# refresh-bio/vclust

Hardware: AMD Instinct MI355X
Metric: genome pairs/sec through prefilter+align (ani.tsv) (higher is better)
Workload: dtype u64

## Files before the change

### include/vclust_gpu.h

```cpp
#ifndef VCLUST_GPU_H
#define VCLUST_GPU_H

#include <stdint.h>

#ifdef __cplusplus
extern "C" {
#endif

enum {
    VG_OK = 0, VG_EINVAL = -1, VG_EIO = -2, VG_ENODEV = -3, VG_EHIP = -4, VG_ENOMEM = -5,
    VG_EOVERFLOW = -6
};

const char* vg_version(void);
const char* vg_last_error(void);
void        vg_free(void* p);
int vg_device_count(void);
int vg_set_device(int device);
void vg_release_device_memory(void);
int vg_alloc_selftest(const int64_t* sizes, int n_sizes, int cycles);
int vg_copy(void* dst, const void* src, int64_t bytes, int to_host);

typedef struct vg_genomes vg_genomes;

int vg_genomes_load(const char* const* paths, int n_paths, int multisample, int n_threads,
                    vg_genomes** out);
int vg_genomes_load_db_new(const char* const* db_paths, int n_db, const char* const* new_paths, int n_new, int multisample,
                           int n_threads, vg_genomes** out, int* n_db_genomes);
int vg_genomes_from_codes(const uint8_t* codes, const int64_t* offsets, int n_genomes,
                          const char* const* names, vg_genomes** out);
void        vg_genomes_free(vg_genomes* g);
int         vg_genomes_count(const vg_genomes* g);
int64_t     vg_genomes_total_len(const vg_genomes* g);
int         vg_genomes_lengths(const vg_genomes* g, int64_t* out );
const char* vg_genomes_name(const vg_genomes* g, int idx);
int         vg_genomes_codes(const vg_genomes* g, int idx, uint8_t* out);
int vg_genomes_to_device(vg_genomes* g);

typedef struct { uint32_t a, b, shared; } vg_pair_count;

int vg_kmer_shared(vg_genomes* g, int k, double fraction, int shard, int n_shards,
                   uint32_t min_shared, int64_t* set_sizes, vg_pair_count** pairs,
                   int64_t* n_pairs);
int vg_kmer_shared_new(vg_genomes* g, int n_db, int k, double fraction, uint32_t min_shared, int64_t* set_sizes,
                       vg_pair_count** pairs, int64_t* n_pairs);
void vg_set_new_path(int mode);
typedef struct {
    int accepted; int64_t P; int n_passes;
    int levels, total_bits, B1, B2;
    int st_tiles; int64_t n_st; int u_st, g_st;
    int tile32k, narrow, short_rec;
} vg_kmer_geometry_info;
int vg_kmer_geometry(const vg_genomes* g, int k, double fraction, int shard, int n_shards, vg_kmer_geometry_info* info);
int vg_kmer_geometry_at(int64_t padded_positions, int k, vg_kmer_geometry_info* info);
int vg_rowptr_inline_lo(int64_t entries, int64_t n_genomes, uint32_t* inline_lo);
int vg_kmer_set(vg_genomes* g, int idx, int k, double fraction, uint64_t** out, int64_t* n_out);

int vg_write_fltr(const vg_genomes* g, int k, double fraction, int min_kmers, double min_ident,
                  int max_seqs, const int64_t* set_sizes, const vg_pair_count* pairs,
                  int64_t n_pairs, const char* out_path);

int vg_filter_pairs(int k, int min_kmers, double min_ident, const int64_t* set_sizes, int64_t n_genomes,
                    const vg_pair_count* pairs, int64_t n_pairs, vg_pair_count** out, int64_t* n_out);

typedef struct {
    int    k;
    int    min_kmers;
    double min_ident;
    int    batch_size;
    double kmers_fraction;
    int    max_seqs;
    int    num_threads;
    int    verbosity;
    int    is_multifasta;
} vg_prefilter_params;
int vg_prefilter(const char* const* fasta_paths, int n_paths, const char* out_path,
                 const vg_prefilter_params* p);
int vg_prefilter_new(const char* const* db_paths, int n_db_paths, const char* const* new_paths, int n_new_paths,
                     const char* out_path, const vg_prefilter_params* p);
void vg_set_process_ends_after_call(int on);

typedef struct { int mal, msl, mrd, mqd, reg, aw, am, ar; } vg_lz_params;
typedef struct { uint32_t q, r; } vg_task;
typedef struct { uint32_t n_match, aln_len, n_regions; } vg_pair_stat;
typedef struct {
    uint32_t task; int32_t qstart, qend, rstart, rend; int32_t n_match;
} vg_region;

typedef struct { int weak_seed_ratio, anchor_margin, seed_choice; } vg_lz_fit;
void vg_set_lz_fit(const vg_lz_fit* f);

int vg_lz_align(vg_genomes* g, const vg_task* tasks, int64_t n_tasks, const vg_lz_params* p,
                vg_pair_stat* stats, vg_region** regions, int64_t* n_regions);

int vg_lz_prepare(vg_genomes* g, const vg_pair_count* pairs, int64_t n_pairs, const vg_lz_params* p);

int vg_align_order(const vg_genomes* g, int32_t* order );
int vg_read_filter(const vg_genomes* g, const char* path, double thr,
                   vg_pair_count** pairs, int64_t* n_pairs);

int vg_align_tasks(const vg_genomes* g, const vg_pair_count* pairs, int64_t n_pairs,
                   vg_task** tasks, int64_t* n_tasks);
int vg_lz_index_dump(vg_genomes* g, int idx, const vg_lz_params* p,
                     uint32_t** bucket_end, uint32_t** entries, int64_t* n_entries,
                     int* pos_bits, int* tag_bits, int* path);
void vg_set_index_budget(int64_t bytes);
void vg_set_subshards(int n);
void vg_set_range_scan(int mode);
void vg_set_placement_trials(int n);

typedef struct {
    vg_lz_params lz;
    double out_tani, out_gani, out_ani, out_qcov, out_rcov;
    const char* filter_path; double filter_threshold;
    const char* out_aln_path;
    const char* const* out_columns; int n_out_columns;
    int num_threads; int verbosity; int is_multifasta;
} vg_align_params;
int vg_write_ani(const vg_genomes* g, const vg_task* tasks, const vg_pair_stat* stats,
                 int64_t n_tasks, const vg_region* regions, int64_t n_regions,
                 const char* out_path, const vg_align_params* p);
int vg_align(const char* const* fasta_paths, int n_paths, const char* out_path,
             const vg_align_params* p);

int vg_align_new(const char* const* db_paths, int n_db_paths, const char* const* new_paths, int n_new_paths,
                 const char* out_path, const vg_align_params* p);

typedef struct vg_comm vg_comm;
typedef int (*vg_allgather_fn)(void* ctx, const void* send, void* recv, int64_t bytes, int on_device);
int  vg_comm_create(int rank, int world, vg_allgather_fn allgather, void* ctx, vg_comm** out);
int  vg_rccl_unique_id(void* out , int64_t bytes);
int  vg_comm_rccl_create(int rank, int world, const void* unique_id, int64_t id_bytes, vg_comm** out);
void vg_comm_free(vg_comm* c);
int  vg_comm_kind(const vg_comm* c);
int  vg_comm_rccl_ranks(const vg_comm* c);
int  vg_comm_rank(const vg_comm* c);
int  vg_comm_world(const vg_comm* c);
int  vg_comm_selftest(const vg_comm* c, int64_t bytes);
int vg_kmer_shared_sharded(vg_genomes* g, int k, double fraction, uint32_t min_shared, const vg_comm* c,
                           int64_t* set_sizes, vg_pair_count** pairs, int64_t* n_pairs);
int vg_align_owner(const vg_task* tasks, int64_t n_tasks, int n_genomes, int world, int32_t* owner );
int vg_lz_align_sharded(vg_genomes* g, const vg_task* tasks, int64_t n_tasks, const vg_lz_params* p, const vg_comm* c,
                        vg_pair_stat* stats, vg_region** regions, int64_t* n_regions);
int vg_align_pairs_share(const vg_genomes* g, const vg_pair_count* pairs, int64_t n_pairs, int world, int rank,
                         vg_task** tasks, int64_t* n_tasks);
int vg_lz_align_pairs_sharded(vg_genomes* g, const vg_pair_count* pairs, int64_t n_pairs, const vg_lz_params* p, const vg_comm* c,
                              vg_task** tasks, int64_t* n_tasks, vg_pair_stat** stats);
int vg_prefilter_sharded(const char* const* fasta_paths, int n_paths, const char* out_path,
                         const vg_prefilter_params* p, const vg_comm* c);
int vg_align_sharded(const char* const* fasta_paths, int n_paths, const char* out_path,
                     const vg_align_params* p, const vg_comm* c);

enum { VG_CLUSTER_SINGLE = 0, VG_CLUSTER_CDHIT = 1, VG_CLUSTER_UCLUST = 2, VG_CLUSTER_SET_COVER = 3, VG_CLUSTER_COMPLETE = 4, VG_CLUSTER_AVERAGE = 5,
       VG_CLUSTER_MCL = 6  };
typedef struct {
    int algorithm;
    const char* metric;
    double min_tani, min_gani, min_ani, min_qcov, min_rcov, min_len_ratio;
    int max_num_alns;
    int representatives;
    int num_threads; int verbosity;
} vg_cluster_params;
typedef struct {
    int64_t rounds;
    int64_t sweep_objects;
    int64_t n_edges;
} vg_cluster_stats;
int vg_cluster(const char* ani_path, const char* ids_path, const char* out_path, const vg_cluster_params* p);
int vg_cluster_graph(int64_t n_objects, const uint32_t* q, const uint32_t* r, const double* w, int64_t n_edges,
                     int algorithm, int32_t* label, int32_t* representative, vg_cluster_stats* stats);

typedef struct {
    int64_t rounds, sweep_objects, n_edges;
    int64_t n_prior, n_new;
    int64_t joined_prior, joined_new, founded;
    int64_t prior_merged;
} vg_cluster_update_stats;
int vg_cluster_update_graph(int64_t n_objects, const uint32_t* q, const uint32_t* r, const double* w, int64_t n_rows,
                            int algorithm, const int32_t* prior_rep, int32_t* label, int32_t* representative,
                            vg_cluster_update_stats* stats);
int vg_cluster_update(const char* ani_path, const char* ids_path, const char* prior_path, int prior_is_repr,
                      const char* out_path, const vg_cluster_params* p, vg_cluster_update_stats* stats);

typedef struct {
    int64_t rounds;
// ... 132 lines not shown
```

### vclust_amd/_lib.py

```python
import ctypes as C
import pathlib

PKG_DIR = pathlib.Path(__file__).resolve().parent
LIB_PATH = PKG_DIR / 'libvclust_gpu.so'


class VclustGpuError(RuntimeError):
    def __init__(self, code, msg):
        super().__init__(f'libvclust_gpu error {code}: {msg}')
        self.code = code


class PairCount(C.Structure):
    _fields_ = [('a', C.c_uint32), ('b', C.c_uint32), ('shared', C.c_uint32)]


class Task(C.Structure):
    _fields_ = [('q', C.c_uint32), ('r', C.c_uint32)]


class PairStat(C.Structure):
    _fields_ = [('n_match', C.c_uint32), ('aln_len', C.c_uint32), ('n_regions', C.c_uint32)]


# ... 65 lines not shown

class MclStats(C.Structure):
    _fields_ = [(name, C.c_int64) for name in ('iterations', 'converged', 'n_edges', 'nnz', 'max_row_seen', 'lds_rows', 'spill_rows')] + [('chaos', C.c_uint64)]


class DedupParams(C.Structure):
    _fields_ = [('gzip_level', C.c_int), ('num_threads', C.c_int), ('verbosity', C.c_int)]


class DedupStats(C.Structure):
    _fields_ = [('records', C.c_int64), ('unique', C.c_int64), ('removed', C.c_int64), ('reverse', C.c_int64),
                ('rounds', C.c_int64), ('collisions', C.c_int64)]


class DedupOptions(C.Structure):
    _fields_ = [('circular', C.c_int)]


class DedupContainedStats(C.Structure):
    _fields_ = [('passes', C.c_int64), ('positions', C.c_int64), ('hits', C.c_int64), ('candidates', C.c_int64),
                ('verified', C.c_int64), ('slices', C.c_int64)]


class DedupRepeatStats(C.Structure):
    _fields_ = [('with_repeat', C.c_int64), ('repeat_symbols', C.c_int64), ('candidates', C.c_int64), ('equal', C.c_int64),
                ('batches', C.c_int64)]


class KmerGeometry(C.Structure):
    _fields_ = [('accepted', C.c_int), ('P', C.c_int64), ('n_passes', C.c_int),
                ('levels', C.c_int), ('total_bits', C.c_int), ('B1', C.c_int), ('B2', C.c_int),
                ('st_tiles', C.c_int), ('n_st', C.c_int64), ('u_st', C.c_int), ('g_st', C.c_int),
                ('tile32k', C.c_int), ('narrow', C.c_int), ('short_rec', C.c_int)]


class KernelTime(C.Structure):
    _fields_ = [('name', C.c_char * 48), ('total_ms', C.c_double), ('launches', C.c_int64),
                ('bytes', C.c_double)]


ALLGATHER_FN = C.CFUNCTYPE(C.c_int, C.c_void_p, C.c_void_p, C.c_void_p, C.c_int64, C.c_int)

P = C.POINTER
SYMBOLS = {
    'vg_version': (C.c_char_p, []),
    'vg_last_error': (C.c_char_p, []),
    'vg_free': (None, [C.c_void_p]),
    'vg_device_count': (C.c_int, []),
    'vg_set_device': (C.c_int, [C.c_int]),
    'vg_release_device_memory': (None, []),
    'vg_copy': (C.c_int, [C.c_void_p, C.c_void_p, C.c_int64, C.c_int]),
    'vg_alloc_selftest': (C.c_int, [C.POINTER(C.c_int64), C.c_int, C.c_int]),
    'vg_genomes_load': (C.c_int, [P(C.c_char_p), C.c_int, C.c_int, C.c_int, P(C.c_void_p)]),
    'vg_genomes_load_db_new': (C.c_int, [P(C.c_char_p), C.c_int, P(C.c_char_p), C.c_int, C.c_int, C.c_int, P(C.c_void_p), P(C.c_int)]),
    'vg_genomes_from_codes': (C.c_int, [C.c_void_p, C.c_void_p, C.c_int, P(C.c_char_p), P(C.c_void_p)]),
    'vg_genomes_free': (None, [C.c_void_p]),
    'vg_genomes_count': (C.c_int, [C.c_void_p]),
    'vg_genomes_total_len': (C.c_int64, [C.c_void_p]),
    'vg_genomes_lengths': (C.c_int, [C.c_void_p, P(C.c_int64)]),
    'vg_genomes_name': (C.c_char_p, [C.c_void_p, C.c_int]),
    'vg_genomes_codes': (C.c_int, [C.c_void_p, C.c_int, C.c_void_p]),
    'vg_genomes_to_device': (C.c_int, [C.c_void_p]),
    'vg_kmer_shared': (C.c_int, [C.c_void_p, C.c_int, C.c_double, C.c_int, C.c_int, C.c_uint32,
                                 P(C.c_int64), P(P(PairCount)), P(C.c_int64)]),
    'vg_kmer_shared_new': (C.c_int, [C.c_void_p, C.c_int, C.c_int, C.c_double, C.c_uint32, P(C.c_int64), P(P(PairCount)), P(C.c_int64)]),
    'vg_kmer_geometry': (C.c_int, [C.c_void_p, C.c_int, C.c_double, C.c_int, C.c_int, P(KmerGeometry)]),
    'vg_kmer_geometry_at': (C.c_int, [C.c_int64, C.c_int, P(KmerGeometry)]),
    'vg_rowptr_inline_lo': (C.c_int, [C.c_int64, C.c_int64, P(C.c_uint32)]),
    'vg_kmer_set': (C.c_int, [C.c_void_p, C.c_int, C.c_int, C.c_double, P(P(C.c_uint64)), P(C.c_int64)]),
    'vg_filter_pairs': (C.c_int, [C.c_int, C.c_int, C.c_double, C.POINTER(C.c_int64), C.c_int64, C.POINTER(PairCount), C.c_int64,
                                  C.POINTER(C.POINTER(PairCount)), C.POINTER(C.c_int64)]),
    'vg_write_fltr': (C.c_int, [C.c_void_p, C.c_int, C.c_double, C.c_int, C.c_double, C.c_int,
                                P(C.c_int64), P(PairCount), C.c_int64, C.c_char_p]),
    'vg_prefilter': (C.c_int, [P(C.c_char_p), C.c_int, C.c_char_p, P(PrefilterParams)]),
    'vg_prefilter_new': (C.c_int, [P(C.c_char_p), C.c_int, P(C.c_char_p), C.c_int, C.c_char_p, P(PrefilterParams)]),
    'vg_set_process_ends_after_call': (None, [C.c_int]),
    'vg_set_lz_fit': (None, [P(LzFit)]),
    'vg_lz_align': (C.c_int, [C.c_void_p, P(Task), C.c_int64, P(LzParams), P(PairStat),
                              P(P(Region)), P(C.c_int64)]),
    'vg_align_order': (C.c_int, [C.c_void_p, P(C.c_int32)]),
    'vg_read_filter': (C.c_int, [C.c_void_p, C.c_char_p, C.c_double, P(P(PairCount)), P(C.c_int64)]),
    'vg_align_tasks': (C.c_int, [C.c_void_p, P(PairCount), C.c_int64, P(P(Task)), P(C.c_int64)]),
    'vg_lz_prepare': (C.c_int, [C.c_void_p, P(PairCount), C.c_int64, P(LzParams)]),
    'vg_lz_index_dump': (C.c_int, [C.c_void_p, C.c_int, P(LzParams), P(P(C.c_uint32)), P(P(C.c_uint32)), P(C.c_int64),
                                   P(C.c_int), P(C.c_int), P(C.c_int)]),
    'vg_set_index_budget': (None, [C.c_int64]),
    'vg_set_subshards': (None, [C.c_int]),
    'vg_set_range_scan': (None, [C.c_int]),
    'vg_set_new_path': (None, [C.c_int]),
    'vg_set_placement_trials': (None, [C.c_int]),
    'vg_write_ani': (C.c_int, [C.c_void_p, P(Task), P(PairStat), C.c_int64, P(Region), C.c_int64,
                               C.c_char_p, P(AlignParams)]),
    'vg_align': (C.c_int, [P(C.c_char_p), C.c_int, C.c_char_p, P(AlignParams)]),
    'vg_align_new': (C.c_int, [P(C.c_char_p), C.c_int, P(C.c_char_p), C.c_int, C.c_char_p, P(AlignParams)]),
    'vg_comm_create': (C.c_int, [C.c_int, C.c_int, C.c_void_p, C.c_void_p, P(C.c_void_p)]),
    'vg_rccl_unique_id': (C.c_int, [C.c_void_p, C.c_int64]),
    'vg_comm_rccl_create': (C.c_int, [C.c_int, C.c_int, C.c_void_p, C.c_int64, P(C.c_void_p)]),
    'vg_comm_free': (None, [C.c_void_p]),
    'vg_comm_kind': (C.c_int, [C.c_void_p]),
    'vg_comm_rccl_ranks': (C.c_int, [C.c_void_p]),
    'vg_comm_rank': (C.c_int, [C.c_void_p]),
    'vg_comm_world': (C.c_int, [C.c_void_p]),
    'vg_comm_selftest': (C.c_int, [C.c_void_p, C.c_int64]),
    'vg_kmer_shared_sharded': (C.c_int, [C.c_void_p, C.c_int, C.c_double, C.c_uint32, C.c_void_p, P(C.c_int64), P(P(PairCount)), P(C.c_int64)]),
    'vg_align_owner': (C.c_int, [P(Task), C.c_int64, C.c_int, C.c_int, P(C.c_int32)]),
    'vg_align_pairs_share': (C.c_int, [C.c_void_p, P(PairCount), C.c_int64, C.c_int, C.c_int, P(P(Task)), P(C.c_int64)]),
    'vg_lz_align_pairs_sharded': (C.c_int, [C.c_void_p, P(PairCount), C.c_int64, P(LzParams), C.c_void_p, P(P(Task)), P(C.c_int64), P(P(PairStat))]),
    'vg_lz_align_sharded': (C.c_int, [C.c_void_p, P(Task), C.c_int64, P(LzParams), C.c_void_p, P(PairStat), P(P(Region)), P(C.c_int64)]),
    'vg_prefilter_sharded': (C.c_int, [P(C.c_char_p), C.c_int, C.c_char_p, P(PrefilterParams), C.c_void_p]),
    'vg_align_sharded': (C.c_int, [P(C.c_char_p), C.c_int, C.c_char_p, P(AlignParams), C.c_void_p]),
    'vg_cluster': (C.c_int, [C.c_char_p, C.c_char_p, C.c_char_p, P(ClusterParams)]),
    'vg_cluster_graph': (C.c_int, [C.c_int64, P(C.c_uint32), P(C.c_uint32), P(C.c_double), C.c_int64, C.c_int,
                                   P(C.c_int32), P(C.c_int32), P(ClusterStats)]),
    'vg_cluster_update_graph': (C.c_int, [C.c_int64, P(C.c_uint32), P(C.c_uint32), P(C.c_double), C.c_int64, C.c_int, P(C.c_int32),
                                          P(C.c_int32), P(C.c_int32), P(ClusterUpdateStats)]),
    'vg_cluster_update': (C.c_int, [C.c_char_p, C.c_char_p, C.c_char_p, C.c_int, C.c_char_p, P(ClusterParams), P(ClusterUpdateStats)]),
    'vg_cluster_stats_graph': (C.c_int, [C.c_int64, P(C.c_uint32), P(C.c_uint32), P(C.c_double), C.c_int64, P(C.c_int32), C.c_int64,
                                         P(ClusterStat), P(C.c_uint64), P(C.c_uint64), P(C.c_int32)]),
    'vg_cluster_stats_file': (C.c_int, [C.c_char_p, C.c_char_p, C.c_char_p, C.c_int, P(ClusterParams), C.c_char_p]),
    'vg_cluster_linkage_graph': (C.c_int, [C.c_int64, P(C.c_uint32), P(C.c_uint32), P(C.c_double), C.c_int64, P(C.c_int32), P(C.c_int32),
                                           P(C.c_double), P(C.c_int64), P(C.c_int64), P(C.c_int64), P(C.c_int64), P(LinkageStats)]),
    'vg_cluster_levels_graph': (C.c_int, [C.c_int64, P(C.c_uint32), P(C.c_uint32), P(C.c_double), C.c_int64, P(C.c_double), C.c_int,
                                          P(C.c_int32), P(C.c_int32), P(LinkageStats)]),
    'vg_cluster_complete_linkage_graph': (C.c_int, [C.c_int64, P(C.c_uint32), P(C.c_uint32), P(C.c_double), C.c_int64, P(C.c_int32), P(C.c_int32),
                                                    P(C.c_double), P(C.c_int64), P(C.c_int64), P(C.c_int64), P(C.c_int64), P(LinkageStats)]),
    'vg_cluster_complete_levels_graph': (C.c_int, [C.c_int64, P(C.c_uint32), P(C.c_uint32), P(C.c_double), C.c_int64, P(C.c_double), C.c_int,
                                                   P(C.c_int32), P(C.c_int32), P(LinkageStats)]),
    'vg_cluster_average_linkage_graph': (C.c_int, [C.c_int64, P(C.c_uint32), P(C.c_uint32), P(C.c_double), C.c_int64, C.c_double, P(C.c_int32),
                                                   P(C.c_int32), P(C.c_double), P(C.c_uint64), P(C.c_uint64), P(C.c_int64), P(C.c_int64),
                                                   P(C.c_int64), P(C.c_int64), P(LinkageStats)]),
    'vg_cluster_average_levels_graph': (C.c_int, [C.c_int64, P(C.c_uint32), P(C.c_uint32), P(C.c_double), C.c_int64, C.c_double, P(C.c_double),
                                                  C.c_int, P(C.c_int32), P(C.c_int32), P(LinkageStats)]),
    'vg_cluster_average_similarity': (C.c_double, [C.c_uint64, C.c_uint64]),
    'vg_cluster_average_order_selftest': (C.c_int, [P(C.c_uint64), P(C.c_uint32), P(C.c_uint32), P(C.c_uint32), P(C.c_uint32), C.c_int64,
                                                    C.c_int, P(C.c_int8)]),
    'vg_cluster_linkage': (C.c_int, [C.c_char_p, C.c_char_p, C.c_char_p, P(ClusterParams), C.c_char_p, P(C.c_double), C.c_int]),
    'vg_cluster_mcl_graph': (C.c_int, [C.c_int64, P(C.c_uint32), P(C.c_uint32), P(C.c_double), C.c_int64, P(MclParams), P(C.c_int32), P(C.c_int32),
                                       P(P(C.c_int64)), P(P(C.c_int32)), P(P(C.c_uint32)), P(MclStats)]),
    'vg_cluster_mcl': (C.c_int, [C.c_char_p, C.c_char_p, C.c_char_p, P(ClusterParams), P(MclParams), P(MclStats)]),
    'vg_cluster_mcl_set_table_slots': (None, [C.c_int]),
    'vg_deduplicate': (C.c_int, [P(C.c_char_p), C.c_int, P(C.c_char_p), C.c_char_p, C.c_char_p, P(DedupParams)]),
    'vg_dedup_seqs': (C.c_int, [C.c_char_p, P(C.c_int64), C.c_int64, P(C.c_int32), P(C.c_int8), P(DedupStats)]),
    'vg_deduplicate_ex': (C.c_int, [P(C.c_char_p), C.c_int, P(C.c_char_p), C.c_char_p, C.c_char_p, P(DedupParams), P(DedupOptions)]),
    'vg_dedup_seqs_ex': (C.c_int, [C.c_char_p, P(C.c_int64), C.c_int64, P(DedupOptions), P(C.c_int32), P(C.c_int8), P(C.c_int64),
                                   P(DedupStats)]),
    'vg_dedup_set_hash_bits': (None, [C.c_int]),
    'vg_dedup_terminal_repeats': (C.c_int, [C.c_char_p, P(C.c_int64), C.c_int64, C.c_int64, P(C.c_int64)]),
    'vg_dedup_seqs_circular_tr': (C.c_int, [C.c_char_p, P(C.c_int64), C.c_int64, C.c_int64, P(C.c_int32), P(C.c_int8), P(C.c_int64),
                                            P(C.c_int64), P(DedupStats), P(DedupRepeatStats)]),
    'vg_deduplicate_circular_tr': (C.c_int, [P(C.c_char_p), C.c_int, P(C.c_char_p), C.c_char_p, C.c_char_p, P(DedupParams), C.c_int64]),
    'vg_deduplicate_contained': (C.c_int, [P(C.c_char_p), C.c_int, P(C.c_char_p), C.c_char_p, C.c_char_p, P(DedupParams)]),
    'vg_dedup_seqs_contained': (C.c_int, [C.c_char_p, P(C.c_int64), C.c_int64, P(C.c_int32), P(C.c_int8), P(C.c_int64), P(DedupStats),
                                          P(DedupContainedStats)]),
    'vg_dedup_set_anchor_symbols': (None, [C.c_int]),
    'vg_dedup_set_index_positions': (None, [C.c_int64]),
    'vg_synth_plan': (C.c_int, [C.c_void_p, C.c_void_p, C.c_void_p, C.c_int64, C.c_uint64, C.c_double, C.c_double, C.c_int,
                                C.c_int, P(C.c_void_p), P(C.c_void_p), P(C.c_int64)]),
    'vg_profile_enable': (None, [C.c_int]),
    'vg_profile_reset': (None, []),
    'vg_profile_get': (C.c_int, [P(KernelTime), C.c_int]),
}

_lib = None


def load():
# ... 25 lines not shown
```

### vclust_amd/build.py

```python
import os
import pathlib
import shutil
import subprocess
import sys

PKG_DIR = pathlib.Path(__file__).resolve().parent
ROOT = PKG_DIR.parent
CSRC = PKG_DIR / 'csrc'
LIB_PATH = PKG_DIR / 'libvclust_gpu.so'
ORACLE_DIR = ROOT / 'oracle'

SOURCES = ['vg_core.cpp', 'vg_genomes.cpp', 'vg_inflate.cpp', 'vg_io.cpp', 'vg_api.cpp', 'vg_synth.cpp', 'vg_prefilter.hip', 'vg_align.hip', 'vg_dist.hip', 'vg_cluster.hip', 'vg_dedup.hip']


def _hipcc() -> str:
    for cand in (os.environ.get('HIPCC'), shutil.which('hipcc'), '/opt/rocm/bin/hipcc'):
        if cand and pathlib.Path(cand).exists():
            return cand
    raise RuntimeError('hipcc not found (needs ROCm)')


def _stale(target: pathlib.Path, deps) -> bool:
    if not target.exists():
        return True
    t = target.stat().st_mtime
    return any(pathlib.Path(d).stat().st_mtime > t for d in deps)


def build_lib(force: bool = False, verbose: bool = False) -> pathlib.Path:
    srcs = [CSRC / s for s in SOURCES]
    deps = srcs + [CSRC / 'vg_common.h', CSRC / 'vg_window.h', ROOT / 'include' / 'vclust_gpu.h']
    if not force and not _stale(LIB_PATH, deps):
        return LIB_PATH
    obj_dir = PKG_DIR / '_obj'
    obj_dir.mkdir(exist_ok=True)
    hipcc = _hipcc()
    flags = ['--offload-arch=gfx950', '-O3', '-std=c++17', '-fPIC', '-Wall', '-Wno-unused-function',
             '-Wno-unused-result', f'-I{ROOT / "include"}']
    if os.environ.get('VG_LINES') == '1':
        flags.append('-gline-tables-only')
    objs = []
    procs = []
    for s in srcs:
        o = obj_dir / (s.name + '.o')
        objs.append(o)
        if force or _stale(o, [s, CSRC / 'vg_common.h', CSRC / 'vg_window.h', ROOT / 'include' / 'vclust_gpu.h']):
            cmd = [hipcc, *flags, '-x', 'hip', '-c', str(s), '-o', str(o)]
            if verbose:
                print(' '.join(cmd), file=sys.stderr)
            procs.append((s, subprocess.Popen(cmd, stdout=subprocess.PIPE, stderr=subprocess.STDOUT, text=True)))
    for s, p in procs:
        out, _ = p.communicate()
        if p.returncode != 0:
            raise RuntimeError(f'hipcc failed on {s.name}:\n{out}')
        if verbose and out.strip():
            print(out, file=sys.stderr)
    cmd = [hipcc, '--offload-arch=gfx950', '-shared', '-fPIC', '-o', str(LIB_PATH), *map(str, objs), '-lz', '-lpthread', '-ldl']
    r = subprocess.run(cmd, stdout=subprocess.PIPE, stderr=subprocess.STDOUT, text=True)
    if r.returncode != 0:
        raise RuntimeError(f'link failed:\n{r.stdout}')
    return LIB_PATH


def build_oracle(verbose: bool = False) -> pathlib.Path:
    r = subprocess.run(['make', '-C', str(ORACLE_DIR)], stdout=subprocess.PIPE, stderr=subprocess.STDOUT, text=True)
    if r.returncode != 0:
        raise RuntimeError(f'oracle build failed:\n{r.stdout}')
    if verbose:
        print(r.stdout, file=sys.stderr)
    return ORACLE_DIR / '_build' / 'liboracle.so'


if __name__ == '__main__':
    force = '--force' in sys.argv
    print(build_lib(force=force, verbose=True))
    print(build_oracle(verbose=False))
```

### vclust_amd/csrc/vg_align.hip

```cpp
#include "vg_common.h"
#include "vg_window.h"
#include <rocprim/rocprim.hpp>
#include <algorithm>
#include <numeric>
#include <cstring>
#include <memory>
#include <mutex>
#include <optional>

namespace {

constexpr int RR_PAD = 128;

struct ref_desc {
    int64_t rr_w;
    int64_t mask_w;
    int64_t stab;
    int64_t sent;
    int32_t L;
    int32_t n_rr;
    int32_t genome;
    int32_t has_n;
    int32_t pos_bits;
    int32_t tag_bits;
};

struct lz_dev_params { int mal, msl, mrd, mqd, reg, aw, am, ar; int pw_after, pw_miss; int weak_ratio; int margin; int seed_choice; };


__device__ __forceinline__ uint32_t loadm32(const uint32_t* __restrict__ mk, int64_t p) {
    int64_t w = p >> 5; int sh = (int)(p & 31);
    uint64_t m = (uint64_t)mk[w] | ((uint64_t)mk[w + 1] << 32);
    return (uint32_t)(m >> sh);
}
__device__ __forceinline__ uint32_t squeeze16(uint32_t x) {
    x &= 0x55555555u;
    x = (x | (x >> 1)) & 0x33333333u;
    x = (x | (x >> 2)) & 0x0F0F0F0Fu;
    x = (x | (x >> 4)) & 0x00FF00FFu;
    return (x | (x >> 8)) & 0x0000FFFFu;
}
__device__ __forceinline__ uint32_t squeeze(uint64_t x) {
    return squeeze16((uint32_t)x) | (squeeze16((uint32_t)(x >> 32)) << 16);
}
struct planes32 { uint32_t lo, hi; };
__device__ __forceinline__ planes32 planes_of(uint64_t codes) { return { squeeze(codes), squeeze(codes >> 1) }; }

__device__ __forceinline__ planes32 loadp(const uint32_t* __restrict__ pl, int64_t p) {
    const uint32_t off = ((uint32_t)p >> 5) << 3; const uint32_t sh = (uint32_t)p & 31u;
    uint4 v; __builtin_memcpy(&v, (const char*)pl + off, 16);
    asm volatile("" :: "v"(v.w));
    return { __builtin_amdgcn_alignbit(v.z, v.x, sh), __builtin_amdgcn_alignbit(v.w, v.y, sh) };
}
__device__ __forceinline__ uint32_t diff32(const planes32 a, const planes32 b) { return (a.lo ^ b.lo) | (a.hi ^ b.hi); }
__device__ __forceinline__ uint32_t slots(int lo, int hi) {
    if (lo < 0) lo = 0; if (hi > 32) hi = 32;
    if (hi <= lo) return 0u;
    const uint32_t a = (hi == 32) ? ~0u : ((1u << hi) - 1u);
    return a & ~((1u << lo) - 1u);
}

struct pair_ctx {
    const uint32_t* qpl; const uint32_t* qmk; int qlen; int q_has_n;
    const uint32_t* rpl; const uint32_t* rmk; int n_rr; int L; int r_has_n;
};

__device__ __forceinline__ uint32_t mism32(const pair_ctx& c, int qp, int rp, int rlo, int rhi) {
    const int lo = max(-qp, rlo - rp); const int hi = min(c.qlen - qp, rhi - rp);
    if (lo <= 0 && hi >= 32) {
        uint32_t mm = diff32(loadp(c.qpl, qp), loadp(c.rpl, rp));
        if (c.q_has_n) mm |= loadm32(c.qmk, qp);
        if (c.r_has_n) mm |= loadm32(c.rmk, rp);
        return mm;
    }
    const uint32_t ok = slots(lo, hi);
    if (ok == 0) return ~0u;
    const int qs = qp < 0 ? 0 : qp, rs = rp < 0 ? 0 : rp;
    planes32 xq = loadp(c.qpl, qs), xr = loadp(c.rpl, rs);
    if (qp < 0) { xq.lo <<= -qp; xq.hi <<= -qp; }
    if (rp < 0) { xr.lo <<= -rp; xr.hi <<= -rp; }
    uint32_t mm = diff32(xq, xr);
    if (c.q_has_n) { uint32_t sp = loadm32(c.qmk, qs); if (qp < 0) sp <<= -qp; mm |= sp; }
    if (c.r_has_n) { uint32_t sp = loadm32(c.rmk, rs); if (rp < 0) sp <<= -rp; mm |= sp; }
    return mm | ~ok;
// ... 728 lines not shown
            }
            b_lo = b_hi;
        }
        for (uint32_t i = 4u * (uint32_t)tid; i < (uint32_t)nb; i += 4096u) { const uint4 v = make_uint4(tab[i], tab[i + 1], tab[i + 2], tab[i + 3]); __builtin_memcpy(gtab + i, &v, 16); }
        lds_sync();
    }
}

__global__ void __launch_bounds__(256)
k_build_rr(const ref_desc* __restrict__ refs, const int* __restrict__ slot_list, int n_list,
           const int64_t* __restrict__ chunk_off ,
           const uint32_t* __restrict__ gplanes, const uint32_t* __restrict__ nmask, const int64_t* __restrict__ base_off,
           uint32_t* __restrict__ rr_pool, uint32_t* __restrict__ mask_pool) {
    const int64_t total = chunk_off[n_list];
    for (int64_t t = (int64_t)blockIdx.x * blockDim.x + threadIdx.x; t < total; t += (int64_t)gridDim.x * blockDim.x) {
        int lo = 0, hi = n_list - 1;
        while (lo < hi) { int mid = (lo + hi + 1) >> 1; if (chunk_off[mid] <= t) lo = mid; else hi = mid - 1; }
        const ref_desc rd = refs[slot_list[lo]];
        const int64_t ch = t - chunk_off[lo];
        const int64_t g0 = base_off[rd.genome];
        uint32_t pl_lo, pl_hi, m;
        rr_chunk_planes(gplanes + (g0 >> 4), nmask + (g0 >> 5), rd.L, ch, &pl_lo, &pl_hi, &m);
        rr_pool[rd.rr_w + 2 * ch] = pl_lo; rr_pool[rd.rr_w + 2 * ch + 1] = pl_hi;
        mask_pool[rd.mask_w + ch] = m;
    }
}

__global__ void __launch_bounds__(256)
k_index_pass(const ref_desc* __restrict__ refs, const int* __restrict__ slot_list, int n_list, const int64_t* __restrict__ chunk_off,
             const uint32_t* __restrict__ rr_pool, const uint32_t* __restrict__ mask_pool, int mal, int msl, int fill,
             uint32_t* __restrict__ stab_pool,
             uint32_t* __restrict__ sent_pool) {
    const int64_t total = chunk_off[n_list] * 32;
    (void)mal;
    for (int64_t t = (int64_t)blockIdx.x * blockDim.x + threadIdx.x; t < total; t += (int64_t)gridDim.x * blockDim.x) {
        int64_t chunk = t >> 5;
        int lo = 0, hi = n_list - 1;
        while (lo < hi) { int mid = (lo + hi + 1) >> 1; if (chunk_off[mid] <= chunk) lo = mid; else hi = mid - 1; }
        const ref_desc rd = refs[slot_list[lo]];
        const int64_t p = t - chunk_off[lo] * 32;
        if (p >= rd.n_rr) continue;
        const uint32_t* pk = rr_pool + rd.rr_w; const uint32_t* mk = mask_pool + rd.mask_w;
        const planes32 x = loadp(pk, p);
        uint64_t m = (uint64_t)mk[p >> 5] | ((uint64_t)mk[(p >> 5) + 1] << 32);
        m >>= (p & 31);
        if (p + msl <= rd.n_rr && (m & ((1ULL << msl) - 1)) == 0) {
            uint32_t b = bucket_of(x.lo, x.hi, msl);
            uint32_t slot = atomicAdd(&stab_pool[rd.stab + b], 1u);
            if (fill) sent_pool[rd.sent + slot] = (uint32_t)p | (tag_of(x.lo, x.hi, msl, rd.tag_bits) << rd.pos_bits);
        }
    }
}

__global__ void __launch_bounds__(256)
k_scan_tables(const ref_desc* __restrict__ refs, const int* __restrict__ slot_list, int msl,
              uint32_t* __restrict__ stab_pool) {
    __shared__ uint32_t part[256];
    __shared__ uint32_t carry;
    const ref_desc rd = refs[slot_list[blockIdx.x]];
    uint32_t* tab = stab_pool + rd.stab;
    const int64_t n = 1LL << (2 * msl);
    if (threadIdx.x == 0) carry = 0;
    __syncthreads();
    for (int64_t base = 0; base < n; base += 256 * 8) {
        uint32_t v[8]; uint32_t s = 0;
        int64_t i0 = base + (int64_t)threadIdx.x * 8;
        for (int j = 0; j < 8; ++j) { v[j] = (i0 + j < n) ? tab[i0 + j] : 0; s += v[j]; }
        part[threadIdx.x] = s;
        __syncthreads();
        for (int o = 1; o < 256; o <<= 1) {
            uint32_t add = threadIdx.x >= (unsigned)o ? part[threadIdx.x - o] : 0;
            __syncthreads();
            part[threadIdx.x] += add;
            __syncthreads();
        }
        uint32_t excl = part[threadIdx.x] - s + carry;
        for (int j = 0; j < 8; ++j) { if (i0 + j < n) tab[i0 + j] = excl; excl += v[j]; }
        __syncthreads();
        if (threadIdx.x == 255) carry += part[255];
        __syncthreads();
    }
}

struct task_dev { uint32_t q, r_slot, out_idx, pad; };

constexpr int SEG_LOG_CAP = 250;
constexpr int PW_AFTER_EVENT = 32;
struct seg_rec { int i_ev, ev_pos; uint32_t VM, VA, VN; };
constexpr int RCHUNK = 8;
struct region_rec { uint32_t task; int32_t qstart, qend, rstart, rend, n_match; uint32_t k, t; };
static_assert(sizeof(region_rec) == 32, "arena record");

#define PARSE_ARGS \
    const task_dev* __restrict__ tasks, int64_t n_tasks, const ref_desc* __restrict__ refs, \
    const uint32_t* __restrict__ planes, const uint32_t* __restrict__ nmask, const int64_t* __restrict__ base_off, \
    const int64_t* __restrict__ glen, const uint8_t* __restrict__ g_has_n, \
    const uint32_t* __restrict__ rr_pool, const uint32_t* __restrict__ mask_pool, \
    const uint32_t* __restrict__ stab_pool, const uint32_t* __restrict__ sent_pool, \
    lz_dev_params P, vg_pair_stat* __restrict__ stats, \
    region_rec* __restrict__ arena, unsigned long long* __restrict__ arena_cursor, unsigned long long arena_cap
#define PARSE_ARG_NAMES tasks, n_tasks, refs, planes, nmask, base_off, glen, g_has_n, rr_pool, mask_pool, \
    stab_pool, sent_pool, P, stats, arena, arena_cursor, arena_cap

template <int S, bool FAST = false, bool REG = false>
__device__ __forceinline__ void lz_parse_body(PARSE_ARGS) {
    static_assert(!REG || S == 1, "regions are emitted by the one-wave parse (query order)");
    if (FAST) { P.mal = 11; P.msl = 7; P.mrd = 40; P.mqd = 40; P.reg = 35; P.aw = 15; P.am = 7; P.ar = 3; P.weak_ratio = 3; P.margin = 6; P.seed_choice = 3; }
    __shared__ seg_rec s_log[S > 1 ? S * SEG_LOG_CAP : 1];
    __shared__ int s_cnt[4], s_sync_v[4], s_sync_idx[4];
    __shared__ uint32_t s_end[4][3];
    const int lane = threadIdx.x & 63;
    const int w = __builtin_amdgcn_readfirstlane((int)(threadIdx.x >> 6));
    const int64_t per_xcd = gridDim.x / 8;
    const int64_t vblk = (int64_t)(blockIdx.x % 8) * per_xcd + blockIdx.x / 8;
    const int64_t t = (S == 1) ? vblk * 4 + w : vblk;
    if (t >= n_tasks) return;
    const task_dev tk = tasks[t];
    ref_desc rd = refs[tk.r_slot];
    if (FAST) { rd.tag_bits = 8; rd.has_n = 0; }
    pair_ctx c;
    const int64_t qb = base_off[tk.q];
    c.qpl = planes + (qb >> 4); c.qmk = nmask + (qb >> 5); c.qlen = (int)glen[tk.q]; c.q_has_n = FAST ? 0 : g_has_n[tk.q];
    c.rpl = rr_pool + rd.rr_w; c.rmk = mask_pool + rd.mask_w; c.n_rr = rd.n_rr; c.L = rd.L; c.r_has_n = rd.has_n;
    const uint32_t* stab = stab_pool + rd.stab; const uint32_t* sent = sent_pool + rd.sent;

    const int lim = c.qlen - P.mal;
    const int seg_len = (S > 1 && lim >= S * 2048) ? ((((lim + S - 1) / S) + 63) & ~63) : (lim > 0 ? lim : 1);
    const int seg_start = (S > 1) ? min(w * seg_len, lim > 0 ? lim : 0) : 0;
    int phase_end = (S > 1 && w < S - 1) ? min((w + 1) * seg_len, lim) : lim;
    int i = seg_start, lit = 0, pred = 0; bool alive = false;
    int n_events = 0;
    int pw = 64;
    bool synced = false; int sync_v = -1, sync_idx = 0, log_n = 0, look_v = -1, look_cur = 0;
    bool in_region = false; int r_qstart = 0, r_rstart = 0, r_qend = 0, r_rend = -1, r_match = 0, vend = 0;
    int kept_end = seg_start;
    uint32_t M = 0, A = 0, NR = 0;
    unsigned long long chunk_base = 0;

    auto close_region = [&]() {
        if (in_region) {
            int span = r_qend - r_qstart + 1;
            if (span >= P.reg) {
                M += (uint32_t)r_match; A += (uint32_t)span; NR += 1; kept_end = r_qend + 1;
                if (REG) {
                    const uint32_t kk = NR - 1;
                    if ((kk & (RCHUNK - 1)) == 0) {
                        unsigned long long b = 0;
                        if (lane == 0) b = atomicAdd(arena_cursor, (unsigned long long)RCHUNK);
                        chunk_base = ((unsigned long long)(uint32_t)__builtin_amdgcn_readfirstlane((int)(uint32_t)(b >> 32)) << 32) |
                                     (unsigned long long)(uint32_t)__builtin_amdgcn_readfirstlane((int)(uint32_t)b);
                    }
                    const unsigned long long at = chunk_base + (kk & (RCHUNK - 1));
                    if (lane == 0 && at < arena_cap) {
                        region_rec rg; rg.task = tk.out_idx; rg.qstart = r_qstart; rg.qend = r_qend;
                        rg.rstart = r_rstart; rg.rend = r_rend; rg.n_match = r_match; rg.k = kk; rg.t = (uint32_t)t;
                        arena[at] = rg;
                    }
                }
            }
            in_region = false;
        }
    };

    for (int phase = 0; phase < (S > 1 ? 2 : 1); ++phase) {
    while (i < phase_end) {
        const int qi = i + lane;
        int best_len = 0, best_pos = 0; bool hit_close = false;
// ... 173 lines not shown
    }
    if (synced) break;
    }
    if (!synced) close_region();
    if (S > 1) {
        if (lane == 0) { s_end[w][0] = M; s_end[w][1] = A; s_end[w][2] = NR; s_sync_v[w] = sync_v; s_sync_idx[w] = sync_idx; }
        __syncthreads();
        if (threadIdx.x == 0) {
            uint32_t tm = 0, ta = 0, tn = 0, bm = 0, ba = 0, bn = 0; int cur = 0;
            for (;;) {
                tm += s_end[cur][0] - bm; ta += s_end[cur][1] - ba; tn += s_end[cur][2] - bn;
                const int v = s_sync_v[cur];
                if (v < 0) break;
                const seg_rec rc = s_log[v * SEG_LOG_CAP + s_sync_idx[cur]];
                bm = rc.VM; ba = rc.VA; bn = rc.VN & 0x7fffffffu; cur = v;
            }
            vg_pair_stat st; st.n_match = tm; st.aln_len = ta; st.n_regions = tn;
            stats[tk.out_idx] = st;
        }
        return;
    }
    if (REG && (NR & (RCHUNK - 1)) != 0) {
        const uint32_t used = NR & (RCHUNK - 1);
        const unsigned long long at = chunk_base + used + (uint32_t)lane;
        if (used + (uint32_t)lane < (uint32_t)RCHUNK && at < arena_cap) arena[at].task = ~0u;
    }
    if (lane == 0) { vg_pair_stat st; st.n_match = M; st.aln_len = A; st.n_regions = NR; stats[tk.out_idx] = st; }
}

#define PARSE_KERNEL(NAME, S, WAVES, FAST, REG) \
    __global__ void __launch_bounds__(256) __attribute__((amdgpu_waves_per_eu(WAVES, 8))) NAME(PARSE_ARGS) { \
        lz_parse_body<S, FAST, REG>(PARSE_ARG_NAMES); }
PARSE_KERNEL(k_lz_parse, 1, 8, false, false)
PARSE_KERNEL(k_lz_parse_fast, 1, 8, true, false)
PARSE_KERNEL(k_lz_parse_seg, 4, 8, false, false)
PARSE_KERNEL(k_lz_parse_seg_fast, 4, 8, true, false)
PARSE_KERNEL(k_lz_parse_regions, 1, 8, false, true)
PARSE_KERNEL(k_lz_parse_fast_regions, 1, 8, true, true)

__global__ void __launch_bounds__(256)
k_region_counts(const task_dev* __restrict__ tasks, int64_t n_tasks, const vg_pair_stat* __restrict__ stats, unsigned long long* __restrict__ cnt) {
    for (int64_t t = (int64_t)blockIdx.x * blockDim.x + threadIdx.x; t <= n_tasks; t += (int64_t)gridDim.x * blockDim.x)
        cnt[t] = t < n_tasks ? (unsigned long long)stats[tasks[t].out_idx].n_regions : 0ULL;
}
__global__ void __launch_bounds__(256)
k_regions_place(const region_rec* __restrict__ arena, unsigned long long n_slots, const unsigned long long* __restrict__ first,
                unsigned long long n_out, vg_region* __restrict__ out, unsigned int* __restrict__ bad) {
    for (unsigned long long i = (unsigned long long)blockIdx.x * blockDim.x + threadIdx.x; i < n_slots; i += (unsigned long long)gridDim.x * blockDim.x) {
        const region_rec r = arena[i];
        if (r.task == ~0u) continue;
        const unsigned long long at = first[r.t] + r.k;
        if (at >= first[r.t + 1] || at >= n_out) { atomicAdd(bad, 1u); continue; }
        vg_region o; o.task = r.task; o.qstart = r.qstart; o.qend = r.qend; o.rstart = r.rstart; o.rend = r.rend; o.n_match = r.n_match;
        out[at] = o;
    }
}

}

static std::mutex g_fit_mu;
static bool g_fit_set = false;
static vg_lz_fit g_fit{ 3, -1, 3 };
static vg_lz_fit lz_fit_now() {
    std::lock_guard<std::mutex> lk(g_fit_mu);
    if (!g_fit_set) {
        g_fit_set = true;
        if (const char* e = vg_dev_getenv("VG_LZ_WEAK_SEED")) if (*e) g_fit.weak_seed_ratio = atoi(e);
        if (const char* e = vg_dev_getenv("VG_LZ_ANCHOR_MARGIN")) if (*e) g_fit.anchor_margin = atoi(e);
        if (const char* e = vg_dev_getenv("VG_LZ_SEED_CHOICE")) if (*e) g_fit.seed_choice = atoi(e);
        if (g_fit.weak_seed_ratio != 3 || g_fit.anchor_margin >= 0 || g_fit.seed_choice != 3)
            fprintf(stderr, "libvclust_gpu: LZ fit constants changed by developer switches (weak seed ratio %d, anchor margin %d, seed choice %d): results differ from the reference's\n",
                    g_fit.weak_seed_ratio, g_fit.anchor_margin, g_fit.seed_choice);
    }
    return g_fit;
}
extern "C" void vg_set_lz_fit(const vg_lz_fit* f) {
    std::lock_guard<std::mutex> lk(g_fit_mu);
    g_fit_set = true;
    g_fit = f ? *f : vg_lz_fit{ 3, -1, 3 };
}
static bool g_index_budget_set = false;
static int64_t g_index_budget_bytes = [] { const char* e = getenv("VG_INDEX_BUDGET_GB"); const double v = e ? atof(e) : 0.0; g_index_budget_set = v >= 0.0625; return v >= 0.0625 ? (int64_t)(v * 1073741824.0) : (24LL << 30); }();
namespace {
__global__ void __launch_bounds__(256)
k_task_count(const vg_task* __restrict__ tasks, int64_t n_tasks, int n_genomes, const int64_t* __restrict__ len,
             uint32_t* __restrict__ ref_cnt, uint32_t* __restrict__ keys, uint32_t* __restrict__ vals,
             unsigned long long* __restrict__ sums ) {
    unsigned long long sq = 0, sr = 0, mq = 0, bad = 0;
    for (int64_t t = (int64_t)blockIdx.x * blockDim.x + threadIdx.x; t < n_tasks; t += (int64_t)gridDim.x * blockDim.x) {
        const vg_task tk = tasks[t];
        keys[t] = tk.r; vals[t] = (uint32_t)t;
        if (tk.q >= (uint32_t)n_genomes || tk.r >= (uint32_t)n_genomes) { bad = 1; continue; }
        atomicAdd(&ref_cnt[tk.r], 1u);
        const unsigned long long ql = (unsigned long long)len[tk.q];
        sq += ql; sr += (unsigned long long)len[tk.r]; mq = ql > mq ? ql : mq;
    }
    for (int o = 32; o > 0; o >>= 1) {
        sq += __shfl_xor(sq, o); sr += __shfl_xor(sr, o); bad |= __shfl_xor(bad, o);
        const unsigned long long m2 = __shfl_xor(mq, o); mq = m2 > mq ? m2 : mq;
    }
    if ((threadIdx.x & 63) == 0) {
        if (sq) atomicAdd(&sums[0], sq);
        if (sr) atomicAdd(&sums[1], sr);
        if (mq) atomicMax(&sums[2], mq);
        if (bad) atomicOr(&sums[3], 1ULL);
    }
}
__global__ void __launch_bounds__(256)
k_task_records(const vg_task* __restrict__ tasks, const uint32_t* __restrict__ sorted_idx, int64_t n_tasks,
               const uint32_t* __restrict__ ord , task_dev* __restrict__ td) {
    for (int64_t i = (int64_t)blockIdx.x * blockDim.x + threadIdx.x; i < n_tasks; i += (int64_t)gridDim.x * blockDim.x) {
        const uint32_t t = sorted_idx[i];
        const vg_task tk = tasks[t];
        td[i] = { tk.q, ord[tk.r], t, 0u };
    }
}
}

namespace {
struct lz_batch {
    int first_ref = 0, n_refs = 0;
    std::vector<int64_t> chunk_off{ 0 };
    std::vector<int> reg_list, mid_list, small_list, large_list; std::vector<int64_t> large_chunks{ 0 };
    int reg_class_end[6] = {0, 0, 0, 0, 0, 0};
    int64_t rr_words = 0, mask_words = 0, stab_tot = 0, sent_n = 0, scratch_words = 0, stride = 0;
    int nblk_build = 0;
};
struct lz_slot { dbuf<uint32_t> rr_pool, mask_pool, stab_pool, sent_pool, scratch; dbuf<int> d_reg, d_mid, d_small, d_large; dbuf<int64_t> d_lchunk; };
struct lz_plan {
    std::vector<uint32_t> ref_ids;
    std::vector<lz_batch> batches;
    std::vector<ref_desc> all_refs;
    dbuf<ref_desc> d_refs;
    lz_slot slot;
    int64_t budget = 0; int mal = 0, msl = 0; const vg_genomes* g = nullptr; int n_genomes = 0;
    bool batch0_built = false;
};
int64_t lz_batch_budget(const vg_genomes* g, const vg_lz_params* p, const std::vector<uint32_t>& ref_ids);
void lz_plan_references(const vg_genomes* g, const vg_lz_params* p, lz_plan& P);
void lz_plan_alloc(lz_plan& P);
void lz_build_batch(const vg_genomes* g, const vg_lz_params* p, lz_plan& P, size_t bi, hipStream_t sb);
std::mutex g_prep_mu;
std::unique_ptr<lz_plan> g_prepared;
std::unique_ptr<lz_plan> g_plan_cache;
std::unique_ptr<lz_plan> lz_take_plan(std::unique_ptr<lz_plan>& kept, const vg_genomes* g, const vg_lz_params* p, const std::vector<uint32_t>& ref_ids) {
    std::lock_guard<std::mutex> lk(g_prep_mu);
    std::unique_ptr<lz_plan> Q = std::move(kept);
    if (Q && (Q->g != g || Q->mal != p->mal || Q->msl != p->msl || Q->n_genomes != g->n || Q->ref_ids != ref_ids || Q->budget != lz_batch_budget(g, p, ref_ids))) Q.reset();
    return Q;
}
std::unique_ptr<lz_plan> lz_plan_for(const vg_genomes* g, const vg_lz_params* p, const std::vector<uint32_t>& ref_ids, bool* taken_over = nullptr) {
    std::unique_ptr<lz_plan> plan = lz_take_plan(g_plan_cache, g, p, ref_ids);
    if (taken_over) *taken_over = plan != nullptr;
    if (plan) lz_plan_alloc(*plan);
    else {
        plan.reset(new lz_plan);
        plan->g = g; plan->ref_ids = ref_ids;
        lz_plan_references(g, p, *plan);
    }
    return plan;
}
void lz_keep_plan_host_side(std::unique_ptr<lz_plan>& plan) {
    if (!plan || vg_one_shot()) return;
    plan->slot = lz_slot(); plan->d_refs.release();
    plan->batch0_built = false;
    std::lock_guard<std::mutex> lk(g_prep_mu);
    g_plan_cache = std::move(plan);
}
}
void vg_lz_drop_prepared(const vg_genomes* g) {
    std::lock_guard<std::mutex> lk(g_prep_mu);
    if (g_prepared && (!g || g_prepared->g == g)) { (void)hipStreamSynchronize(vg_stream()); g_prepared.reset(); }
    if (g_plan_cache && (!g || g_plan_cache->g == g)) g_plan_cache.reset();
}

namespace {
__global__ void __launch_bounds__(256)
k_genome_planes(const uint32_t* __restrict__ packed, int64_t n_pairs, uint32_t* __restrict__ planes) {
    for (int64_t w = (int64_t)blockIdx.x * blockDim.x + threadIdx.x; w < n_pairs; w += (int64_t)gridDim.x * blockDim.x) {
        uint2 v; __builtin_memcpy(&v, packed + 2 * w, 8);
        const planes32 pl = planes_of((uint64_t)v.x | ((uint64_t)v.y << 32));
        const uint2 o = make_uint2(pl.lo, pl.hi); __builtin_memcpy(planes + 2 * w, &o, 8);
    }
}
}
static std::mutex g_planes_mu;
const uint32_t* vg_genome_planes(const vg_genomes* g, hipStream_t s) {
    std::lock_guard<std::mutex> lk(g_planes_mu);
    hipStream_t lib = vg_stream();
    if (g->d_planes.n != g->d_packed.n || !g->d_planes.p) {
        const size_t words = g->d_packed.n & ~(size_t)1;
        g->d_planes.alloc(g->d_packed.n);
        hipLaunchKernelGGL(k_genome_planes, dim3(grid_for((int64_t)(words / 2))), dim3(256), 0, lib, (const uint32_t*)g->d_packed.p, (int64_t)(words / 2), g->d_planes.p);
    }
    if (s != lib) {
        hipEvent_t e = nullptr;
        VG_HIP(hipEventCreateWithFlags(&e, hipEventDisableTiming));
        VG_HIP(hipEventRecord(e, lib)); VG_HIP(hipStreamWaitEvent(s, e, 0));
        (void)hipEventDestroy(e);
    }
    return g->d_planes.p;
}

namespace {
constexpr int64_t SEGMENT_TASK_LIMIT = 32768;
bool lz_switch_is(const char* name, const char* value) { const char* e = vg_dev_getenv(name); return e && !strcmp(e, value); }
const struct {
    bool two_pass = lz_switch_is("VG_LZ_REGIONS", "two-pass");
    bool general = lz_switch_is("VG_LZ_KERNEL", "general");
    bool lds_build = lz_switch_is("VG_LZ_BUILD", "lds");
    const char* segments = vg_dev_getenv("VG_LZ_SEGMENTS");
    const char* arena = vg_dev_getenv("VG_LZ_ARENA");
} g_sw{};

void lz_check_params(const vg_lz_params* p) {
    if (p->mal < 8 || p->mal > 31 || p->msl < 4 || p->msl > 12 || p->msl > p->mal) throw vg_error(VG_EINVAL, "mal must be 8..31, msl 4..12 and <= mal");
}
void lz_check_lengths(const vg_genomes* g, int first, int end) {
    for (int i = first; i < end; ++i) if (g->len[(size_t)i] > (1 << 29)) throw vg_error(VG_EOVERFLOW, "genome longer than 2^29 bases");
}

struct lz_tasks {
    dbuf<task_dev> d_tasks;
    std::vector<int64_t> ref_first;
    std::vector<uint32_t> ref_ids;
    int64_t q_max = 0; double q_sum = 0, bytes_alg_all = 0;
    std::vector<task_dev> td;
};
lz_tasks lz_group_tasks(const vg_genomes* g, const vg_task* tasks, int64_t n_tasks, bool host_copy, hipStream_t s) {
    lz_tasks T;
    T.ref_first.assign((size_t)g->n + 1, 0);
    T.d_tasks.alloc((size_t)n_tasks);
    dbuf<vg_task> d_raw((size_t)n_tasks); d_raw.upload(tasks, (size_t)n_tasks, s);
    dbuf<uint32_t> d_cnt((size_t)g->n), d_keys((size_t)n_tasks), d_vals((size_t)n_tasks), d_keys2((size_t)n_tasks), d_vals2((size_t)n_tasks);
    dbuf<unsigned long long> d_sums(4);
    d_cnt.zero(s); d_sums.zero(s);
    hipLaunchKernelGGL(k_task_count, dim3(grid_for(n_tasks, 256, 512)), dim3(256), 0, s,
                       (const vg_task*)d_raw.p, n_tasks, g->n, g->d_len.p, d_cnt.p, d_keys.p, d_vals.p, d_sums.p);
    std::vector<uint32_t> cnt((size_t)g->n); unsigned long long sums[4];
    d_cnt.download(cnt.data(), cnt.size(), s); d_sums.download(sums, 4, s);
    const unsigned id_bits = bit_width((uint64_t)std::max(g->n, 1) - 1, 1);
    with_temp_storage([&](void* tmp, size_t& tb) {
        return rocprim::radix_sort_pairs(tmp, tb, d_keys.p, d_keys2.p, d_vals.p, d_vals2.p, (size_t)n_tasks, 0u, id_bits, s); });
    VG_HIP(hipStreamSynchronize(s));
    if (sums[3]) throw vg_error(VG_EINVAL, "task id out of range");
    std::vector<uint32_t> ord((size_t)g->n, 0);
    for (int i = 0; i < g->n; ++i) {
        if (cnt[(size_t)i]) { ord[(size_t)i] = (uint32_t)T.ref_ids.size(); T.ref_ids.push_back((uint32_t)i); }
        T.ref_first[(size_t)i + 1] = T.ref_first[(size_t)i] + cnt[(size_t)i];
    }
    T.q_max = (int64_t)sums[2]; T.q_sum = (double)sums[0];
    T.bytes_alg_all = ((double)sums[0] + (double)sums[1]) / 4.0 + 20.0 * (double)n_tasks;
    dbuf<uint32_t> d_ord((size_t)g->n); d_ord.upload(ord.data(), ord.size(), s);
    hipLaunchKernelGGL(k_task_records, dim3(grid_for(n_tasks)), dim3(256), 0, s, (const vg_task*)d_raw.p, (const uint32_t*)d_vals2.p, n_tasks,
                       (const uint32_t*)d_ord.p, T.d_tasks.p);
    if (host_copy) { T.td.resize((size_t)n_tasks); T.d_tasks.download(T.td.data(), T.td.size(), s); }
    VG_HIP(hipStreamSynchronize(s));
    return T;
}

struct lz_kernel_params { lz_dev_params P; bool fast; };
lz_kernel_params lz_device_params(const vg_genomes* g, const vg_lz_params* p) {
    const int pw_after = PW_AFTER_EVENT, pw_miss = 64;
    const vg_lz_fit fit = lz_fit_now();
    const int weak_ratio = std::max(0, std::min(fit.weak_seed_ratio, 1000));
    const int margin = fit.anchor_margin >= 0 ? std::min(fit.anchor_margin, 1000) : p->msl - 1;
    const int seed_choice = fit.seed_choice == 1 ? 1 : 3;
    const lz_dev_params P{ p->mal, p->msl, p->mrd, p->mqd, p->reg, p->aw, p->am, p->ar, pw_after, pw_miss, weak_ratio, margin, seed_choice };
    bool fast = !g_sw.general && weak_ratio == 3 && margin == 6 && seed_choice == 3 && p->mal == 11 && p->msl == 7 && p->mrd == 40 && p->mqd == 40 && p->reg == 35 && p->aw == 15 && p->am == 7 && p->ar == 3;
    for (int i = 0; fast && i < g->n; ++i) if (g->has_n[(size_t)i] || g->len[(size_t)i] >= (1 << 22)) fast = false;
    return { P, fast };
}

struct lz_range { int64_t pos, end; double bytes_alg; int64_t q_max, q_sum; };
lz_range lz_task_range(const lz_batch& B, const lz_tasks& T, int64_t n_tasks) {
    const size_t ri_end = (size_t)B.first_ref + (size_t)B.n_refs;
    const int64_t pos = T.ref_first[T.ref_ids[(size_t)B.first_ref]], end = ri_end < T.ref_ids.size() ? T.ref_first[T.ref_ids[ri_end]] : n_tasks;
    return { pos, end, T.bytes_alg_all * (double)(end - pos) / (double)n_tasks, T.q_max, (int64_t)(T.q_sum * (double)(end - pos) / (double)n_tasks) };
}

struct lz_call {
    const vg_genomes* g; const uint32_t* d_planes; const task_dev* d_tasks; const lz_plan* plan; lz_dev_params P; bool fast;
    vg_pair_stat* d_stats; int64_t n_tasks; hipStream_t s;
};
using parse_fn = void (*)(PARSE_ARGS);
parse_fn lz_parse_kernel(bool segments, bool fast, bool regions) {
    if (regions) return fast ? k_lz_parse_fast_regions : k_lz_parse_regions;
    if (segments) return fast ? k_lz_parse_seg_fast : k_lz_parse_seg;
    return fast ? k_lz_parse_fast : k_lz_parse;
}
void lz_launch_parse(const lz_call& c, const lz_range& R, bool segments, bool fast,
                     region_rec* arena = nullptr, unsigned long long* cursor = nullptr, unsigned long long cap = 0) {
    const int64_t nt = R.end - R.pos;
    const int64_t nblk = segments ? (nt + 7) / 8 * 8 : ((nt + 3) / 4 + 7) / 8 * 8;
    const parse_fn kern = lz_parse_kernel(segments, fast, arena != nullptr);
    const vg_genomes* g = c.g; const lz_slot& L = c.plan->slot;
    hipLaunchKernelGGL(kern, dim3((unsigned)nblk), dim3(256), 0, c.s, c.d_tasks + R.pos, nt, c.plan->d_refs.p, c.d_planes, g->d_nmask.p,
                       g->d_base_off.p, g->d_len.p, g->d_has_n.p, L.rr_pool.p, L.mask_pool.p, L.stab_pool.p,
                       L.sent_pool.p, c.P, c.d_stats, arena, cursor, cap);
}
void lz_batch_rows(const lz_call& c, const lz_range& R) {
    const int64_t nt = R.end - R.pos;
    vg_prof_scope ps("lz_parse", R.bytes_alg);
    const bool uneven = R.q_max * nt > 3 * R.q_sum;
    const bool segments = g_sw.segments ? atoi(g_sw.segments) > 1 : ((c.n_tasks <= SEGMENT_TASK_LIMIT && nt <= SEGMENT_TASK_LIMIT) || uneven);
    lz_launch_parse(c, R, segments && nt < (1LL << 31), c.fast);
}

unsigned long long lz_parse_and_place(const lz_call& c, const lz_range& R, bool fast, unsigned long long cap, const char* misplaced, std::vector<vg_region>& h_regions) {
    const int64_t nt = R.end - R.pos; hipStream_t s = c.s;
    dbuf<unsigned long long> d_cur(1), d_first((size_t)nt + 1);
    dbuf<unsigned int> d_bad(1);
    dbuf<region_rec> d_arena((size_t)cap);
    std::optional<vg_prof_scope> ps; ps.emplace("lz_parse", R.bytes_alg);
    d_cur.zero(s); d_bad.zero(s);
    lz_launch_parse(c, R, false, fast, d_arena.p, d_cur.p, cap);
    ps.emplace("lz_regions_place", 0);
    hipLaunchKernelGGL(k_region_counts, dim3(grid_for(nt + 1)), dim3(256), 0, s, c.d_tasks + R.pos, nt, (const vg_pair_stat*)c.d_stats, d_first.p);
    with_temp_storage([&](void* tmp, size_t& tb) {
        return rocprim::exclusive_scan(tmp, tb, d_first.p, d_first.p, 0ULL, (size_t)nt + 1, rocprim::plus<unsigned long long>(), s); });
    ps.reset();
    unsigned long long used = 0, nr = 0;
    d_cur.download(&used, 1, s);
    VG_HIP(hipMemcpyAsync(&nr, d_first.p + nt, sizeof nr, hipMemcpyDeviceToHost, s));
    VG_HIP(hipStreamSynchronize(s));
    if (used > cap || !nr) return used;
    dbuf<vg_region> d_regions((size_t)nr);
    ps.emplace("lz_regions_place", (double)used * 32.0 + (double)nr * 24.0);
    hipLaunchKernelGGL(k_regions_place, dim3(grid_for((int64_t)used)), dim3(256), 0, s, (const region_rec*)d_arena.p, used,
                       (const unsigned long long*)d_first.p, nr, d_regions.p, d_bad.p);
    ps.reset();
    unsigned int bad = 0; d_bad.download(&bad, 1, s);
    const size_t at = h_regions.size();
    h_regions.resize(at + (size_t)nr);
    d_regions.download(h_regions.data() + at, (size_t)nr, s);
    VG_HIP(hipStreamSynchronize(s));
    if (bad) throw vg_error(VG_EHIP, misplaced);
    return used;
}
void lz_batch_regions(const lz_call& c, const lz_range& R, std::vector<vg_region>& h_regions) {
    const int64_t nt = R.end - R.pos;
    unsigned long long cap = (unsigned long long)nt * RCHUNK + (unsigned long long)(R.q_sum / 256) + 1024;
    if (const long long first = g_sw.arena ? atoll(g_sw.arena) : 0LL; first > 0) cap = (unsigned long long)first;
    size_t fr = 0, tot = 0;
    if (hipMemGetInfo(&fr, &tot) == hipSuccess && fr > 0)
        cap = std::min(cap, std::max<unsigned long long>((unsigned long long)nt * RCHUNK / 4 + 1024, (unsigned long long)(fr / 8) / sizeof(region_rec)));
    else (void)hipGetLastError();
    const char* misplaced = "internal error: region records of the LZ parse disagree with its rows";
    const unsigned long long used = lz_parse_and_place(c, R, c.fast, cap, misplaced, h_regions);
    if (used > cap && lz_parse_and_place(c, R, c.fast, used, misplaced, h_regions) > used)
        throw vg_error(VG_EHIP, "internal error: the region arena of the LZ parse overflowed twice");
}
void lz_batch_two_pass(const lz_call& c, const lz_range& R, const std::vector<task_dev>& td, std::vector<vg_pair_stat>& first_pass, std::vector<vg_region>& h_regions) {
    { vg_prof_scope ps("lz_parse", R.bytes_alg); lz_launch_parse(c, R, false, c.fast); }
    std::vector<vg_pair_stat> h_stats((size_t)c.n_tasks);
    vg_download_bytes(h_stats.data(), c.d_stats, h_stats.size() * sizeof(vg_pair_stat), c.s);
    VG_HIP(hipStreamSynchronize(c.s));
    if (first_pass.empty()) first_pass.resize((size_t)c.n_tasks);
    unsigned long long chunks = 0;
    for (int64_t t = R.pos; t < R.end; ++t) {
        const uint32_t oi = td[(size_t)t].out_idx;
        first_pass[oi] = h_stats[oi];
        chunks += (h_stats[oi].n_regions + RCHUNK - 1) / RCHUNK;
    }
    if (chunks && lz_parse_and_place(c, R, false, chunks * RCHUNK, "internal error: the region pass and the counting pass of the LZ parse disagree", h_regions) > chunks * RCHUNK)
        throw vg_error(VG_EHIP, "internal error: the region pass of the LZ parse overflowed the arena sized from the counting pass");
}
}

extern "C" int vg_lz_align(vg_genomes* g, const vg_task* tasks, int64_t n_tasks, const vg_lz_params* p,
                           vg_pair_stat* stats, vg_region** regions, int64_t* n_regions) {
    VG_API_BEGIN
    if (!g || (!tasks && n_tasks) || !p || (!stats && n_tasks)) throw vg_error(VG_EINVAL, "vg_lz_align: null argument");
    lz_check_params(p);
    if (p->aw < 1 || p->aw > 32 || p->ar < 1 || p->ar > 16 || p->am < 0 || p->mrd < 0 || p->mqd < 0 || p->reg < 0)
        throw vg_error(VG_EINVAL, "aw must be 1..32, ar 1..16");
    if (p->mqd > 2000) throw vg_error(VG_EINVAL, "mqd must be <= 2000 (one wave scores a literal run of at most 2 048 symbols)");
    vg_require_device();
    int rc = vg_genomes_to_device(g); if (rc) return rc;
    hipStream_t s = vg_stream();
    vg_host_mark("vg_lz_align: enter");
    const uint32_t* d_planes = vg_genome_planes(g, s);

    if (regions) { *regions = nullptr; if (n_regions) *n_regions = 0; }
    if (n_tasks == 0) return VG_OK;
    lz_check_lengths(g, 0, g->n);
    if (n_tasks >= (1LL << 32)) throw vg_error(VG_EOVERFLOW, "more than 2^32 - 1 ordered pairs in one call: split the task list");
    const bool want_regions = regions != nullptr, two_pass = want_regions && g_sw.two_pass;

    const lz_tasks T = lz_group_tasks(g, tasks, n_tasks, two_pass, s);
    vg_host_mark("lz: tasks grouped");
    const lz_kernel_params K = lz_device_params(g, p);
    dbuf<vg_pair_stat> d_stats((size_t)n_tasks);
    std::unique_ptr<lz_plan> plan = lz_take_plan(g_prepared, g, p, T.ref_ids);
    if (!plan) plan = lz_plan_for(g, p, T.ref_ids);
    std::vector<lz_range> ranges;
    for (const lz_batch& B : plan->batches) ranges.push_back(lz_task_range(B, T, n_tasks));
    vg_host_mark("lz: batches planned");

    const lz_call c{ g, d_planes, T.d_tasks.p, plan.get(), K.P, K.fast, d_stats.p, n_tasks, s };
    std::vector<vg_region> h_regions;
    std::vector<vg_pair_stat> first_pass;
    for (size_t bi = 0; bi < ranges.size(); ++bi) {
        if (!(bi == 0 && plan->batch0_built)) lz_build_batch(g, p, *plan, bi, s);
        if (!want_regions) lz_batch_rows(c, ranges[bi]);
        else if (two_pass) lz_batch_two_pass(c, ranges[bi], T.td, first_pass, h_regions);
        else lz_batch_regions(c, ranges[bi], h_regions);
    }
    vg_host_mark("lz: launched");
    vg_deferred_start();
    VG_HIP(hipStreamSynchronize(s));
    VG_HIP(hipGetLastError());
    vg_host_mark("lz: kernels done");
    d_stats.download(stats, (size_t)n_tasks, s);
    VG_HIP(hipStreamSynchronize(s));
    vg_host_mark("lz: rows downloaded");
    if (want_regions) {
        for (int64_t t = 0; t < n_tasks && !first_pass.empty(); ++t)
            if (stats[t].n_regions != first_pass[(size_t)t].n_regions || stats[t].n_match != first_pass[(size_t)t].n_match || stats[t].aln_len != first_pass[(size_t)t].aln_len)
                throw vg_error(VG_EHIP, "internal error: the region pass and the counting pass of the LZ parse disagree on task " + std::to_string(t));
        vg_region* o = (vg_region*)malloc(sizeof(vg_region) * std::max<size_t>(1, h_regions.size()));
        if (!o) throw vg_error(VG_ENOMEM, "out of host memory");
        if (!h_regions.empty()) memcpy(o, h_regions.data(), sizeof(vg_region) * h_regions.size());
        *regions = o; if (n_regions) *n_regions = (int64_t)h_regions.size();
    }
    lz_keep_plan_host_side(plan);
    VG_API_END
}

namespace {
int64_t lz_ref_need(const vg_genomes* g, const vg_lz_params* p, uint32_t r, int64_t* chunks_out) {
    const int64_t stab_n = 1LL << (2 * p->msl);
    const int64_t n_rr = 2 * g->len[r] + 1;
    const int64_t chunks = (n_rr + RR_PAD + 31) / 32 + 2;
    if (chunks_out) *chunks_out = chunks;
    return chunks * 12 + (stab_n + n_rr) * 4;
}
int64_t lz_batch_budget(const vg_genomes* g, const vg_lz_params* p, const std::vector<uint32_t>& ref_ids) {
    int64_t batch_budget = g_index_budget_bytes;
    if (!g_index_budget_set && vg_one_shot()) {
        static const double gb = [] { const char* e = getenv("VG_ONESHOT_INDEX_GB"); const double v = e ? atof(e) : 0.0; return v >= 0.0625 ? v : 6.0; }();
        batch_budget = (int64_t)(gb * 1073741824.0);
    } else if (!g_index_budget_set) {
        int64_t all = 0;
        for (size_t ri = 0; ri < ref_ids.size() && all <= 2 * batch_budget; ++ri) all += lz_ref_need(g, p, ref_ids[ri], nullptr);
        if (all <= 2 * batch_budget) batch_budget = std::max(batch_budget, all);
    }
    return batch_budget;
}
void lz_plan_references(const vg_genomes* g, const vg_lz_params* p, lz_plan& P) {
    hipStream_t s = vg_stream();
    const std::vector<uint32_t>& ref_ids = P.ref_ids;
    const int64_t stab_n = 1LL << (2 * p->msl);
    P.mal = p->mal; P.msl = p->msl; P.g = g; P.n_genomes = g->n;
    const int64_t batch_budget = P.budget = lz_batch_budget(g, p, ref_ids);
    std::vector<lz_batch>& batches = P.batches;
    std::vector<ref_desc>& all_refs = P.all_refs;
    all_refs.assign(ref_ids.size(), ref_desc{});
    for (size_t ri = 0; ri < ref_ids.size();) {
        batches.emplace_back();
        lz_batch& B = batches.back();
        B.first_ref = (int)ri;
        int64_t bytes = 0;
        B.chunk_off.reserve(ref_ids.size() - ri + 1); B.reg_list.reserve(ref_ids.size() - ri);
        const int tag_want = 2 * (p->mal - p->msl);
        while (ri < ref_ids.size()) {
            const uint32_t r = ref_ids[ri];
            const int64_t L = g->len[r]; const int64_t n_rr = 2 * L + 1;
            int64_t chunks = 0; const int64_t need = lz_ref_need(g, p, r, &chunks);
            if (B.n_refs > 0 && bytes + need > batch_budget) break;
            ref_desc& rd = all_refs[ri];
            rd.rr_w = B.rr_words; rd.mask_w = B.mask_words; rd.stab = B.stab_tot; rd.sent = B.sent_n;
            rd.L = (int32_t)L; rd.n_rr = (int32_t)n_rr; rd.genome = (int32_t)r; rd.has_n = g->has_n[r];
            rd.pos_bits = n_rr <= 2 ? 1 : 64 - __builtin_clzll((unsigned long long)(n_rr - 1));
            rd.tag_bits = std::max(0, std::min({ tag_want, 14, 32 - rd.pos_bits }));
            B.rr_words += chunks * 2; B.mask_words += chunks; B.stab_tot += stab_n; B.sent_n += n_rr;
            B.chunk_off.push_back(B.chunk_off.back() + chunks);
            bytes += need; ++B.n_refs; ++ri;
        }
        const int n_refs = B.n_refs;
        for (int i = 0; i < n_refs; ++i) {
            const int gi = B.first_ref + i;
            const bool small = all_refs[(size_t)gi].n_rr <= (1 << 21) && p->msl <= 7;
            if (small && all_refs[(size_t)gi].n_rr <= REG_MAX_RR && !g_sw.lds_build) B.reg_list.push_back(gi);
            else if (small && all_refs[(size_t)gi].n_rr <= MID_MAX_RR && !g_sw.lds_build) B.mid_list.push_back(gi);
            else if (small) B.small_list.push_back(gi);
            else { B.large_list.push_back(gi); B.large_chunks.push_back(B.large_chunks.back() + (B.chunk_off[(size_t)i + 1] - B.chunk_off[(size_t)i])); }
        }
        auto longest_first = [&](std::vector<int>& list) {
            int32_t mn = INT32_MAX, mx = 0;
            for (int i : list) { mn = std::min(mn, all_refs[(size_t)i].n_rr); mx = std::max(mx, all_refs[(size_t)i].n_rr); }
            if (!list.empty() && (int64_t)mx * 4 > (int64_t)mn * 5 && (int64_t)(mx - mn) <= 8 * (int64_t)list.size() + 65536) {
                std::vector<int64_t> at((size_t)(mx - mn) + 2, 0);
                for (int i : list) at[(size_t)(mx - all_refs[(size_t)i].n_rr) + 1]++;
                for (size_t b = 1; b < at.size(); ++b) at[b] += at[b - 1];
                std::vector<int> sorted(list.size());
                for (int i : list) sorted[(size_t)at[(size_t)(mx - all_refs[(size_t)i].n_rr)]++] = i;
                list.swap(sorted);
            } else if (!list.empty() && (int64_t)mx * 4 > (int64_t)mn * 5) {
                std::vector<uint64_t> keyed(list.size());
                for (size_t i = 0; i < keyed.size(); ++i) keyed[i] = ((uint64_t)(0x7fffffffu - (uint32_t)all_refs[(size_t)list[i]].n_rr) << 32) | (uint32_t)list[i];
                std::sort(keyed.begin(), keyed.end());
                for (size_t i = 0; i < keyed.size(); ++i) list[i] = (int)(uint32_t)keyed[i];
            }
        };
        longest_first(B.reg_list); longest_first(B.mid_list); longest_first(B.small_list);
        {
            std::vector<int> by_class[6];
            for (int i : B.reg_list) {
                const int trips = (all_refs[(size_t)i].n_rr + 256 + 4095) / 4096;
                const int cls = trips > 20 ? 0 : trips > 16 ? 1 : trips > 12 ? 2 : trips > 8 ? 3 : trips > 4 ? 4 : 5;
                by_class[cls].push_back(i);
            }
            B.reg_list.clear();
            for (int c = 0; c < 6; ++c) { B.reg_list.insert(B.reg_list.end(), by_class[c].begin(), by_class[c].end()); B.reg_class_end[c] = (int)B.reg_list.size(); }
        }
        if (!B.small_list.empty()) {
            int64_t max_rr = 0; for (int i : B.small_list) max_rr = std::max<int64_t>(max_rr, all_refs[(size_t)i].n_rr);
            B.nblk_build = (int)std::min<size_t>(B.small_list.size(), 512);
            B.stride = (max_rr + 63) / 64 * 64;
            B.scratch_words = (int64_t)B.nblk_build * B.stride * 3;
        }
    }
    vg_host_mark("lz plan: batches cut");
    lz_plan_alloc(P);
}
void lz_plan_alloc(lz_plan& P) {
    hipStream_t s = vg_stream();
    std::vector<lz_batch>& batches = P.batches;
    std::vector<ref_desc>& all_refs = P.all_refs;
    P.d_refs.alloc(std::max<size_t>(1, all_refs.size()));
    if (!all_refs.empty()) P.d_refs.upload(all_refs.data(), all_refs.size(), s);
    vg_host_mark("lz plan: descriptors queued");
    size_t m_rr = 0, m_mask = 0, m_stab = 1, m_sent = 0, m_scr = 1, m_reg = 1, m_mid = 1, m_small = 1, m_large = 1, m_lch = 1;
    for (auto& B : batches) {
        m_rr = std::max(m_rr, (size_t)B.rr_words); m_mask = std::max(m_mask, (size_t)B.mask_words);
        m_stab = std::max(m_stab, (size_t)B.stab_tot); m_sent = std::max(m_sent, (size_t)B.sent_n); m_scr = std::max(m_scr, (size_t)B.scratch_words);
        m_reg = std::max(m_reg, B.reg_list.size()); m_mid = std::max(m_mid, B.mid_list.size()); m_small = std::max(m_small, B.small_list.size()); m_large = std::max(m_large, B.large_list.size());
        m_lch = std::max(m_lch, B.large_chunks.size());
    }
    lz_slot& L = P.slot;
    L.rr_pool.alloc(m_rr + 8); L.mask_pool.alloc(m_mask + 8); L.stab_pool.alloc(m_stab); L.sent_pool.alloc(m_sent + 4);
    L.scratch.alloc(m_scr); L.d_reg.alloc(m_reg); L.d_mid.alloc(m_mid); L.d_small.alloc(m_small); L.d_large.alloc(m_large); L.d_lchunk.alloc(m_lch);
}
void lz_build_batch(const vg_genomes* g, const vg_lz_params* p, lz_plan& P, size_t bi, hipStream_t sb) {
    lz_batch& B = P.batches[bi];
    lz_slot& L = P.slot;
    dbuf<ref_desc>& d_refs = P.d_refs;
    if (!B.reg_list.empty()) L.d_reg.upload(B.reg_list.data(), B.reg_list.size(), sb);
    if (!B.mid_list.empty()) L.d_mid.upload(B.mid_list.data(), B.mid_list.size(), sb);
    if (!B.small_list.empty()) L.d_small.upload(B.small_list.data(), B.small_list.size(), sb);
    if (!B.large_list.empty()) { L.d_large.upload(B.large_list.data(), B.large_list.size(), sb); L.d_lchunk.upload(B.large_chunks.data(), B.large_chunks.size(), sb); }
    const int64_t total_chunks = B.chunk_off.back();
    const uint32_t* gpl = vg_genome_planes(g, sb);
    vg_prof_scope ps("lz_build_index", (double)total_chunks * 32 * (0.375 + 0.375 + 4), sb);
    if (!B.large_list.empty()) VG_HIP(hipMemsetAsync(L.stab_pool.p, 0, (size_t)B.stab_tot * sizeof(uint32_t), sb));
    if (!B.reg_list.empty()) {
        auto launch = [&](auto kern, int first, int end) {
            if (end > first) hipLaunchKernelGGL(kern, dim3((unsigned)std::min(end - first, 512)), dim3(1024), 0, sb, d_refs.p, L.d_reg.p + first,
                                                end - first, gpl, g->d_nmask.p, g->d_base_off.p, L.rr_pool.p, L.mask_pool.p, p->msl, L.stab_pool.p, L.sent_pool.p);
        };
        const int* ce = B.reg_class_end;
        launch(k_build_index_reg<24>, 0, ce[0]); launch(k_build_index_reg<20>, ce[0], ce[1]); launch(k_build_index_reg<16>, ce[1], ce[2]);
        launch(k_build_index_reg<12>, ce[2], ce[3]); launch(k_build_index_reg<8>, ce[3], ce[4]); launch(k_build_index_reg<4>, ce[4], ce[5]);
    }
    if (!B.mid_list.empty()) {
        hipLaunchKernelGGL(k_build_index_mid, dim3((unsigned)std::min<size_t>(B.mid_list.size(), 512)), dim3(1024), 0, sb, d_refs.p, L.d_mid.p,
                           (int)B.mid_list.size(), gpl, g->d_nmask.p, g->d_base_off.p, L.rr_pool.p, L.mask_pool.p, p->msl,
                           L.stab_pool.p, L.sent_pool.p);
    }
    if (!B.small_list.empty()) {
        hipLaunchKernelGGL(k_build_index_lds, dim3(B.nblk_build), dim3(1024), 0, sb, d_refs.p, L.d_small.p, (int)B.small_list.size(),
                           gpl, g->d_nmask.p, g->d_base_off.p, L.rr_pool.p, L.mask_pool.p, p->mal, p->msl,
                           L.stab_pool.p, L.sent_pool.p, L.scratch.p, B.stride);
    }
    if (!B.large_list.empty()) {
        const int nl = (int)B.large_list.size(); const int64_t lc = B.large_chunks.back();
        hipLaunchKernelGGL(k_build_rr, dim3(grid_for(lc)), dim3(256), 0, sb, d_refs.p, L.d_large.p, nl, L.d_lchunk.p, gpl,
                           g->d_nmask.p, g->d_base_off.p, L.rr_pool.p, L.mask_pool.p);
        hipLaunchKernelGGL(k_index_pass, dim3(grid_for(lc * 32)), dim3(256), 0, sb, d_refs.p, L.d_large.p, nl, L.d_lchunk.p, L.rr_pool.p,
                           L.mask_pool.p, p->mal, p->msl, 0, L.stab_pool.p, L.sent_pool.p);
        hipLaunchKernelGGL(k_scan_tables, dim3(nl), dim3(256), 0, sb, d_refs.p, L.d_large.p, p->msl, L.stab_pool.p);
        hipLaunchKernelGGL(k_index_pass, dim3(grid_for(lc * 32)), dim3(256), 0, sb, d_refs.p, L.d_large.p, nl, L.d_lchunk.p, L.rr_pool.p,
                           L.mask_pool.p, p->mal, p->msl, 1, L.stab_pool.p, L.sent_pool.p);
    }
}
}

extern "C" int vg_lz_prepare(vg_genomes* g, const vg_pair_count* pairs, int64_t n_pairs, const vg_lz_params* p) {
    VG_API_BEGIN
    if (!g || (!pairs && n_pairs) || !p) throw vg_error(VG_EINVAL, "vg_lz_prepare: null argument");
    lz_check_params(p);
    vg_require_device();
    int rc = vg_genomes_to_device(g); if (rc) return rc;
    vg_lz_drop_prepared(nullptr);
    if (n_pairs == 0) return VG_OK;
    lz_check_lengths(g, 0, g->n);
    std::vector<uint8_t> is_ref((size_t)g->n, 0);
    for (int64_t i = 0; i < n_pairs; ++i) {
        if (pairs[i].a >= (uint32_t)g->n || pairs[i].b >= (uint32_t)g->n) throw vg_error(VG_EINVAL, "pair id out of range");
        is_ref[pairs[i].a] = 1; is_ref[pairs[i].b] = 1;
    }
    std::vector<uint32_t> ref_ids;
    for (int i = 0; i < g->n; ++i) if (is_ref[(size_t)i]) ref_ids.push_back((uint32_t)i);
    vg_host_mark("lz prepare: references listed");
    bool taken_over = false;
    std::unique_ptr<lz_plan> plan = lz_plan_for(g, p, ref_ids, &taken_over);
    vg_host_mark(taken_over ? "lz prepare: plan of the last call taken over" : "lz prepare: planned");
    lz_build_batch(g, p, *plan, 0, vg_stream());
    plan->batch0_built = true;
    vg_host_mark("lz: first batch of indexes queued");
    std::lock_guard<std::mutex> lk(g_prep_mu);
    g_prepared = std::move(plan);
    VG_API_END
}

extern "C" int vg_lz_index_dump(vg_genomes* g, int idx, const vg_lz_params* p, uint32_t** bucket_end, uint32_t** entries,
                                int64_t* n_entries, int* pos_bits, int* tag_bits, int* path) {
    VG_API_BEGIN
    if (!g || !p || !bucket_end || !entries || !n_entries || !pos_bits || !tag_bits || !path) throw vg_error(VG_EINVAL, "vg_lz_index_dump: null argument");
    *bucket_end = nullptr; *entries = nullptr; *n_entries = 0;
    lz_check_params(p);
    vg_require_device();
    int rc = vg_genomes_to_device(g); if (rc) return rc;
    if (idx < 0 || idx >= g->n) throw vg_error(VG_EINVAL, "genome id out of range");
    lz_check_lengths(g, idx, idx + 1);
    hipStream_t s = vg_stream();
    lz_plan plan;
    plan.g = g; plan.ref_ids.assign(1, (uint32_t)idx);
    lz_plan_references(g, p, plan);
    lz_build_batch(g, p, plan, 0, s);
    const lz_batch& B = plan.batches.at(0);
    const ref_desc& rd = plan.all_refs.at(0);
    const size_t stab_n = (size_t)1 << (2 * p->msl);
    std::vector<uint32_t> tab(stab_n);
    plan.slot.stab_pool.download(tab.data(), stab_n, s);
    VG_HIP(hipStreamSynchronize(s));
    VG_HIP(hipGetLastError());
    const int64_t n = (int64_t)tab[stab_n - 1];
    if (n > (int64_t)rd.n_rr) throw vg_error(VG_EHIP, "internal error: the bucket table ends behind the reference's entry pool");
    uint32_t* tb = (uint32_t*)malloc(sizeof(uint32_t) * stab_n);
    uint32_t* en = (uint32_t*)malloc(sizeof(uint32_t) * std::max<size_t>(1, (size_t)n));
    if (!tb || !en) { free(tb); free(en); throw vg_error(VG_ENOMEM, "out of host memory"); }
    memcpy(tb, tab.data(), sizeof(uint32_t) * stab_n);
    if (n) { vg_download_bytes(en, plan.slot.sent_pool.p + rd.sent, (size_t)n * sizeof(uint32_t), s); (void)hipStreamSynchronize(s); }
    *bucket_end = tb; *entries = en; *n_entries = n; *pos_bits = rd.pos_bits; *tag_bits = rd.tag_bits;
    if (!B.reg_list.empty()) { int c = 0; while (c < 5 && B.reg_class_end[c] == 0) ++c; *path = c; }
    else *path = !B.mid_list.empty() ? 6 : !B.small_list.empty() ? 7 : 8;
    VG_API_END
}

extern "C" void vg_set_index_budget(int64_t bytes) { if (bytes > (64 << 20)) { g_index_budget_bytes = bytes; g_index_budget_set = true; } }

namespace { __global__ void k_warm_align() {} }
void vg_warm_align(hipStream_t s) { hipLaunchKernelGGL(k_warm_align, dim3(1), dim3(64), 0, s); }
```

### vclust_amd/csrc/vg_io.cpp

```cpp
#include "vg_common.h"
#include <cmath>
#include <math.h>
#include <stdio.h>
#include <stdlib.h>
#include <string.h>
#include <algorithm>
#include <unordered_map>
#include <mutex>
#include <numeric>
#include <charconv>
#include <string_view>
#include <fcntl.h>
#include <sys/mman.h>
#include <sys/stat.h>
#include <unistd.h>

double vg_ani_shorter(int64_t shared, int64_t na, int64_t nb, int k) {
    int64_t mn = std::min(na, nb);
    if (mn <= 0 || shared <= 0) return 0.0;
    double j = (double)shared / (double)mn;
    return 1.0 + log(2.0 * j / (1.0 + j)) / (double)k;
}

static int fmt_num_exact(double x, char* buf) {
    for (int prec = 1; prec <= 6; ++prec) {
        char t[64];
        snprintf(t, sizeof t, "%.*g", prec, x);
        if (strtod(t, nullptr) == x) { strcpy(buf, t); return (int)strlen(buf); }
    }
    bool neg = x < 0; double ax = neg ? -x : x;
    char full[400];
    snprintf(full, sizeof full, "%.150f", ax);
    std::string digits; int int_len = 0; bool seen_dot = false;
    for (char* c = full; *c; ++c) { if (*c == '.') { seen_dot = true; continue; } digits.push_back(*c); if (!seen_dot) ++int_len; }
    size_t first = 0; while (first < digits.size() && digits[first] == '0') ++first;
    size_t keep = std::min(digits.size(), first + 6);
    bool up = keep < digits.size() && digits[keep] >= '5';
    digits.resize(keep);
    if (up) {
        int j = (int)keep - 1;
        while (j >= 0 && digits[j] == '9') { digits[j] = '0'; --j; }
        if (j >= 0) digits[j]++; else { digits.insert(digits.begin(), '1'); ++int_len; }
    }
    std::string out = neg ? "-" : "";
    if ((int)digits.size() <= int_len) { out += digits; out.append(int_len - digits.size(), '0'); }
    else { out += digits.substr(0, int_len); out.push_back('.'); out += digits.substr(int_len); }
    strcpy(buf, out.c_str());
    return (int)out.size();
}

int vg_fmt_num(double x, char* buf) {
    static const double P10[] = { 1e0, 1e1, 1e2, 1e3, 1e4, 1e5, 1e6, 1e7, 1e8, 1e9, 1e10, 1e11, 1e12, 1e13, 1e14, 1e15, 1e16, 1e17, 1e18 };
    if (!(x > 1e-12 && x < 1e6)) return fmt_num_exact(x, buf);
    int e = 0;
    if (x >= 1.0) { while (e < 6 && x >= P10[e + 1]) ++e; }
    else { e = -1; while (e > -13 && x < 1.0 / P10[-e]) --e; }
    const int k = 5 - e;
    const double y = (k >= 0) ? x * P10[k] : x / P10[-k];
    const double fl = floor(y); const double fr = y - fl;
    if (!(y >= 1e5 && y < 999999.0)) return fmt_num_exact(x, buf);
    if (fr < 1e-6 || fr > 1.0 - 1e-6 || (fr > 0.5 - 1e-6 && fr < 0.5 + 1e-6)) return fmt_num_exact(x, buf);
    long d = (long)fl + (fr > 0.5 ? 1 : 0);
    char dig[8]; for (int i = 5; i >= 0; --i) { dig[i] = (char)('0' + d % 10); d /= 10; }
    int o = 0;
    if (e >= 0) {
        for (int i = 0; i <= e; ++i) buf[o++] = dig[i];
        if (e < 5) { buf[o++] = '.'; for (int i = e + 1; i < 6; ++i) buf[o++] = dig[i]; }
    } else {
        buf[o++] = '0'; buf[o++] = '.';
        for (int i = 0; i < -e - 1; ++i) buf[o++] = '0';
        for (int i = 0; i < 6; ++i) buf[o++] = dig[i];
    }
    buf[o] = 0;
    return o;
}

int vg_fmt_len_ratio(int64_t a, int64_t b, char* buf) {
    if (a == b) { strcpy(buf, "1"); return 1; }
    return snprintf(buf, 32, "%.4f", (double)std::min(a, b) / (double)std::max(a, b));
}

void vg_write_file(const char* path, const std::vector<std::string_view>& parts) {
    struct closer { void operator()(FILE* f) const { fclose(f); } };
// ... 192 lines not shown
    for (; d < colon; ++d) { if (*d < '0' || *d > '9') { ok = false; break; } ci = ci * 10 + (*d - '0'); }
    if (!ok) ci = atol(std::string(q, colon).c_str());
    ci -= 1;
    static const double p10[16] = { 1, 1e1, 1e2, 1e3, 1e4, 1e5, 1e6, 1e7, 1e8, 1e9, 1e10, 1e11, 1e12, 1e13, 1e14, 1e15 };
    uint64_t m = 0; int nd = 0, frac = -1; bool plain = colon + 1 < fe;
    for (const char* x = colon + 1; x < fe && plain; ++x) {
        if (*x >= '0' && *x <= '9') { m = m * 10 + (uint64_t)(*x - '0'); ++nd; if (frac >= 0) ++frac; }
        else if (*x == '.' && frac < 0) frac = 0; else plain = false;
    }
    val = plain && nd <= 15 ? (double)m / p10[frac < 0 ? 0 : frac] : atof(std::string(colon + 1, fe).c_str());
    return true;
}
void filter_rows(const text_file& f, const char* body, size_t lo, size_t hi, const std::vector<int64_t>& col_id, name_lookup& lookup,
                 double thr, std::vector<vg_pair_count>& out) {
    const vg_genomes* g = lookup.g;
    auto behind = [&](const char* nl) { return nl < f.end() ? nl + 1 : nl; };
    auto line_start = [&](size_t at) { return at == 0 ? body : behind(f.line_end(body + at - 1)); };
    const char* a = line_start(lo); const char* const stop = body + hi < f.end() ? line_start(hi) : f.end();
    int64_t guess = lo == 0 ? 0 : -1;
    bool first_row = lo > 0;
    while (a < stop) {
        const char* nl = f.line_end(a);
        const char* q = a; const char* const e = nl > a && nl[-1] == '\r' ? nl - 1 : nl;
        a = behind(nl);
        const char* c = (const char*)memchr(q, ',', (size_t)(e - q)); if (!c) continue;
        const std::string_view name(q, (size_t)(c - q));
        if (first_row) {
            first_row = false;
            const int64_t est = (int64_t)((double)g->n * (double)(a - body) / (double)std::max<size_t>(1, (size_t)(f.end() - body)));
            for (int64_t d = 0; d <= 4096 && guess < 0; ++d)
                for (int64_t cand : { est + d, est - d }) if (lookup.is(cand, name)) { guess = cand; break; }
        }
        const int64_t row = lookup(name, guess);
        if (row >= 0) guess = row + 1;
        for (q = c + 1; q < e;) {
            const char* n2 = (const char*)memchr(q, ',', (size_t)(e - q)); const char* fe = n2 ? n2 : e;
            long ci; double val;
            if (filter_cell(q, fe, ci, val) && row >= 0 && ci >= 0 && ci < (long)col_id.size() && col_id[(size_t)ci] >= 0 && col_id[(size_t)ci] != row && val >= thr) {
                const uint32_t x = (uint32_t)row, y = (uint32_t)col_id[(size_t)ci];
                out.push_back({ std::max(x, y), std::min(x, y), 0 });
            }
            if (!n2) break;
            q = n2 + 1;
        }
    }
}
void order_couples(std::vector<vg_pair_count>& v, int n) {
    if ((int64_t)v.size() > 4 * (int64_t)n) {
        std::vector<vg_pair_count> tmp(v.size()); std::vector<int64_t> at((size_t)n + 1);
        for (int pass = 0; pass < 2; ++pass) {
            std::fill(at.begin(), at.end(), 0);
            for (const auto& e : v) at[(size_t)(pass ? e.a : e.b) + 1]++;
            for (int i = 0; i < n; ++i) at[(size_t)i + 1] += at[(size_t)i];
            for (const auto& e : v) tmp[(size_t)at[(size_t)(pass ? e.a : e.b)]++] = e;
            v.swap(tmp);
        }
    } else
        std::sort(v.begin(), v.end(), [](const vg_pair_count& x, const vg_pair_count& y) { return x.a != y.a ? x.a < y.a : x.b < y.b; });
    v.erase(std::unique(v.begin(), v.end(), [](const vg_pair_count& x, const vg_pair_count& y) { return x.a == y.a && x.b == y.b; }), v.end());
}
}

extern "C" int vg_read_filter(const vg_genomes* g, const char* path, double thr, vg_pair_count** pairs, int64_t* n_pairs) {
    VG_API_BEGIN
    if (!g || !pairs || !n_pairs) throw vg_error(VG_EINVAL, "vg_read_filter: null argument");
    std::vector<vg_pair_count> v;
    if (!path) {
        for (uint32_t a = 1; a < (uint32_t)g->n; ++a) for (uint32_t b = 0; b < a; ++b) v.push_back({ a, b, 0 });
    } else {
        const text_file f(path, "filter ");
        name_lookup lookup{ g };
        const char* hdr_end = f.line_end(f.p);
        const std::vector<int64_t> col_id = filter_columns(std::string_view(f.p, (size_t)((hdr_end > f.p && hdr_end[-1] == '\r' ? hdr_end - 1 : hdr_end) - f.p)), lookup);
        const char* body = hdr_end < f.end() ? hdr_end + 1 : hdr_end;
        const int n_thr = std::max(1, std::min(vg_host_threads(), 16));
        std::vector<std::vector<vg_pair_count>> part((size_t)n_thr);
        vg_parallel_chunks((int64_t)(f.end() - body), n_thr, [&](int64_t lo, int64_t hi, int t) { filter_rows(f, body, (size_t)lo, (size_t)hi, col_id, lookup, thr, part[(size_t)t]); });
        for (auto& pv : part) v.insert(v.end(), pv.begin(), pv.end());
        order_couples(v, g->n);
    }
    auto o = host_array<vg_pair_count>(v.size());
    if (!v.empty()) memcpy(o.get(), v.data(), sizeof(vg_pair_count) * v.size());
    *pairs = o.release(); *n_pairs = (int64_t)v.size();
    VG_API_END
}

extern "C" int vg_align_tasks(const vg_genomes* g, const vg_pair_count* pairs, int64_t n_pairs,
                              vg_task** tasks, int64_t* n_tasks) {
    return vg_align_tasks_perm(g, pairs, n_pairs, tasks, n_tasks, nullptr);
}
int vg_align_tasks_perm(const vg_genomes* g, const vg_pair_count* pairs, int64_t n_pairs,
                        vg_task** tasks, int64_t* n_tasks, uint32_t* perm) {
    VG_API_BEGIN
    if (!g || (!pairs && n_pairs) || !tasks || !n_tasks) throw vg_error(VG_EINVAL, "vg_align_tasks: null argument");
    if (perm && n_pairs >= (1LL << 32)) throw vg_error(VG_EOVERFLOW, "more than 2^32 pairs");
    vg_host_mark("align_tasks: enter");
    vg_length_order(g);
    vg_host_mark("align_tasks: length order");
    const std::vector<int32_t>& order = g->len_order; const std::vector<int32_t>& rank = g->len_rank;
    struct rp { int32_t lo, hi; uint32_t idx; };
    auto couple = [&](int64_t i) {
        if (pairs[i].a >= (uint32_t)g->n || pairs[i].b >= (uint32_t)g->n) throw vg_error(VG_EINVAL, "pair id out of range");
        const int32_t x = rank[pairs[i].a], y = rank[pairs[i].b];
        return rp{ std::min(x, y), std::max(x, y), (uint32_t)i };
    };
    auto o = host_array<vg_task>(2 * (size_t)n_pairs);
    vg_task* const row = o.get();
    auto emit = [&](int64_t i, const rp& c) {
        row[2 * i] = { (uint32_t)order[(size_t)c.hi], (uint32_t)order[(size_t)c.lo] };
        row[2 * i + 1] = { (uint32_t)order[(size_t)c.lo], (uint32_t)order[(size_t)c.hi] };
        if (perm) perm[i] = c.idx;
    };
    if (n_pairs >= (1 << 21) && vg_host_threads() > 1) {
        const int T = std::max(2, std::min(vg_host_threads(), 16));
        const int64_t ng = std::max<int64_t>(1, g->n);
        std::vector<rp, no_init_alloc<rp>> v, tmp; v.resize((size_t)n_pairs); tmp.resize((size_t)n_pairs);
        std::vector<std::vector<int64_t>> cnt((size_t)T, std::vector<int64_t>((size_t)T + 1, 0));
        auto bucket_of = [&](int32_t lo) { return (int)((int64_t)lo * T / ng); };
        vg_parallel_chunks(n_pairs, T, [&](int64_t a, int64_t b, int t) {
            for (int64_t i = a; i < b; ++i) { v[(size_t)i] = couple(i); cnt[(size_t)t][(size_t)bucket_of(v[(size_t)i].lo)]++; }
        });
        std::vector<int64_t> b_first((size_t)T + 1, 0);
        { int64_t run = 0; for (int bk = 0; bk < T; ++bk) { b_first[(size_t)bk] = run; for (int t = 0; t < T; ++t) { const int64_t c = cnt[(size_t)t][(size_t)bk]; cnt[(size_t)t][(size_t)bk] = run; run += c; } } b_first[(size_t)T] = run; }
        vg_parallel_chunks(n_pairs, T, [&](int64_t a, int64_t b, int t) {
            for (int64_t i = a; i < b; ++i) tmp[(size_t)cnt[(size_t)t][(size_t)bucket_of(v[(size_t)i].lo)]++] = v[(size_t)i];
        });
        vg_parallel_for(T, T, [&](int64_t bk) {
            std::sort(tmp.begin() + b_first[(size_t)bk], tmp.begin() + b_first[(size_t)bk + 1], [](const rp& x, const rp& y) { return x.lo != y.lo ? x.lo < y.lo : (x.hi != y.hi ? x.hi < y.hi : x.idx < y.idx); });
            for (int64_t i = b_first[(size_t)bk]; i < b_first[(size_t)bk + 1]; ++i) emit(i, tmp[(size_t)i]);
        });
    } else {
        std::vector<rp> v((size_t)n_pairs), tmp((size_t)n_pairs);
        std::vector<int64_t> at_lo((size_t)g->n + 1, 0), at_hi((size_t)g->n + 1, 0);
        for (int64_t i = 0; i < n_pairs; ++i) { v[(size_t)i] = couple(i); at_lo[(size_t)v[(size_t)i].lo + 1]++; at_hi[(size_t)v[(size_t)i].hi + 1]++; }
        for (int key = 0; key < g->n; ++key) { at_lo[(size_t)key + 1] += at_lo[(size_t)key]; at_hi[(size_t)key + 1] += at_hi[(size_t)key]; }
        for (int64_t i = 0; i < n_pairs; ++i) tmp[(size_t)at_hi[(size_t)v[(size_t)i].hi]++] = v[(size_t)i];
        for (int64_t i = 0; i < n_pairs; ++i) v[(size_t)at_lo[(size_t)tmp[(size_t)i].lo]++] = tmp[(size_t)i];
        for (int64_t i = 0; i < n_pairs; ++i) emit(i, v[(size_t)i]);
    }
    vg_host_mark("align_tasks: done");
    *tasks = o.release(); *n_tasks = 2 * n_pairs;
    VG_API_END
}

extern "C" int vg_write_ani(const vg_genomes* g, const vg_task* tasks, const vg_pair_stat* stats, int64_t n_tasks,
                            const vg_region* regions, int64_t n_regions, const char* out_path, const vg_align_params* p) {
    VG_API_BEGIN
    if (!g || (!tasks && n_tasks) || (!stats && n_tasks) || !out_path || !p) throw vg_error(VG_EINVAL, "vg_write_ani: null argument");
    if (n_tasks & 1) throw vg_error(VG_EINVAL, "vg_write_ani: tasks must come in (q,r),(r,q) couples");
    enum column { QIDX, RIDX, QUERY, REFERENCE, TANI, GANI, ANI, QCOV, RCOV, NUM_ALNS, LEN_RATIO, QLEN, RLEN, NT_MATCH, NT_MISMATCH };
    constexpr int N_COLUMNS = NT_MISMATCH + 1;
    static const char* const known[N_COLUMNS] = { "qidx", "ridx", "query", "reference", "tani", "gani", "ani", "qcov", "rcov", "num_alns",
                                                  "len_ratio", "qlen", "rlen", "nt_match", "nt_mismatch" };
    std::vector<column> columns;
    std::string head;
    for (int c = 0; c < p->n_out_columns; ++c) {
        const char* const* kn = std::find_if(known, known + N_COLUMNS, [&](const char* x) { return !strcmp(x, p->out_columns[c]); });
        if (kn == known + N_COLUMNS) throw vg_error(VG_EINVAL, std::string("unknown output column ") + p->out_columns[c]);
        columns.push_back((column)(kn - known));
        if (c) head += '\t';
        head += *kn;
    }
    head += '\n';
    for (int64_t t = 0; t < n_tasks; ++t)
        if (tasks[t ^ 1].q != tasks[t].r || tasks[t ^ 1].r != tasks[t].q) throw vg_error(VG_EINVAL, "vg_write_ani: task couple mismatch");
    vg_length_order(g);
// ... 361 lines not shown
```

### vclust_amd/csrc/vg_prefilter.hip

```cpp
#include "vg_common.h"
#include <functional>
#include <map>
#include <mutex>
#include <optional>
#include <rocprim/rocprim.hpp>
#include <algorithm>
#include <cmath>
#include <cstring>

namespace {

constexpr uint64_t SENT = ~0ULL;
constexpr uint32_t SCRAMBLE32 = 0x9E3779B1u;
__host__ __device__ __forceinline__ uint64_t scramble_key(uint64_t cano, int k) {
    const uint32_t L = (uint32_t)cano & ((1u << k) - 1u);
    const uint32_t H = (uint32_t)(cano >> k);
    return ((uint64_t)(H ^ ((L * SCRAMBLE32) >> (32 - k))) << k) | L;
}
__host__ __device__ __forceinline__ uint64_t unscramble_key(uint64_t key, int k) { return scramble_key(key, k); }
constexpr uint32_t DUP_BIT = 0x80000000u;
__device__ __forceinline__ uint32_t rowptr_inline(uint32_t partner) { return 0xFFFFFFFFu - partner; }
__device__ __forceinline__ uint32_t rowptr_partner_of_rs(uint32_t rs) { return 0xFFFFFFFEu - rs; }

__device__ __forceinline__ uint64_t mix64(uint64_t x) {
// ... 2265 lines not shown
    vg_host_mark("buckets: enter");
    pass_timer index_timer(in.index_ms, s);
    bucket_run R{ g, k, dense, in, ix, d_kept, s };
    const level1 opened = open_bucket_run(R, A, clear_rows_aside);
    if (opened != level1::records) return opened == level1::empty;
    const bucket_geometry& G = R.G;
    R.boff.alloc((size_t)G.nbk + 1);
    if (G.levels == 2) level2(R);
    else {
        VG_HIP(hipMemcpyAsync(R.boff.p, R.d_off1.p, ((size_t)G.nb1 + 1) * sizeof(uint32_t), hipMemcpyDeviceToDevice, s));
        R.f_rec = R.a_rec.p;
    }
    bucket_kernels(R);
    return true;
}
static bool index_by_buckets(vg_genomes* g, int k, double fraction, int shard, int n_shards, bool dense_src, const pass_inputs& in, kmer_index& ix) {
    hipStream_t s = vg_stream();
    const int n = g->n; const int64_t P = g->padded_total(); bool ok = false;
    dbuf<int> kept_b((size_t)n); kept_b.zero(s);
    const kmer_args A = make_kmer_args(g, k, 1.0, dense_src ? shard : 0, dense_src ? n_shards : 1);
    if (dense_src) {
        if (P < (1LL << 32)) {
            ix.n_rows_info = P;
            ok = build_index_buckets(g, k, true, A, kept_b.p, in, ix);
            if (ok) kept_b.download(ix.kept.data(), (size_t)n, s);
        }
    } else {
        extract_kmers(g, k, fraction, shard, n_shards, in, ix.si);
        ix.nv = ix.si.n_valid; ix.n_rows_info = std::max<int64_t>(ix.nv, 1);
        ok = build_index_buckets(g, k, false, A, nullptr, in, ix);
        if (ok) ix.si.kept.download(ix.kept.data(), (size_t)n, s);
    }
    if (ok) { ix.d_dups.download(ix.dups.data(), (size_t)n, s); VG_HIP(hipStreamSynchronize(s)); }
    vg_host_mark("index built");
    return ok;
}
static void index_by_radix(vg_genomes* g, int k, double fraction, int shard, int n_shards, const pass_inputs& in, kmer_index& ix) {
    hipStream_t s = vg_stream(); const int n = g->n;
    sorted_index& si = ix.si; dbuf<uint32_t>& rowinfo = ix.rowinfo; dbuf<uint32_t>& gen = ix.gen; dbuf<int>& d_dups = ix.d_dups;
    rowinfo.release(); gen.release(); ix.arena.release();
    d_dups.zero(s);
    si = sorted_index();
    extract_kmers(g, k, fraction, shard, n_shards, in, si);
    prefix_sort(si, k);
    const int64_t nv = ix.nv = si.n_valid;
    ix.n_rows_info = si.compact ? std::max<int64_t>(nv, 1) : g->padded_total();
    if (2 * si.spare64.n >= (size_t)ix.n_rows_info) rowinfo.view(reinterpret_cast<uint32_t*>(si.spare64.p), (size_t)ix.n_rows_info);
    else rowinfo.alloc((size_t)ix.n_rows_info);
    VG_HIP(hipMemsetAsync(rowinfo.p, 0, (size_t)ix.n_rows_info * sizeof(uint32_t), s));
    const compact_map cmap{ si.compact ? si.goff.p : nullptr, si.compact ? si.cblk.p : nullptr };
    gen = si.spare32.n >= (size_t)std::max<int64_t>(nv, 1) + 4 ? std::move(si.spare32) : dbuf<uint32_t>((size_t)std::max<int64_t>(nv, 1) + 4);
    ix.inline_lo = rowptr_inline_lo((uint64_t)gen.n, n);
    constexpr unsigned int LONG_CAP = 1u << 16;
    dbuf<int64_t> long_list(LONG_CAP); dbuf<unsigned int> d_nlong(1), d_full(1); d_nlong.zero(s); d_full.zero(s);
    if (nv > 0) {
        vg_prof_scope ps("index_runs", (double)nv * (8 + 4 + 4 + 8));
        hipLaunchKernelGGL(k_group_runs, dim3(grid_for(nv, GS_TILE)), dim3(256), 0, s, si.keys.p, si.pos.p, g->d_blk2g.p, g->align_shift, nv,
                           si.low_bit, gen.p, rowinfo.p, cmap, d_dups.p, long_list.p, d_nlong.p, LONG_CAP, ix.inline_lo);
    }
    unsigned int n_long = 0, need_full = 0;
    d_nlong.download(&n_long, 1, s); si.kept.download(ix.kept.data(), (size_t)n, s); d_dups.download(ix.dups.data(), (size_t)n, s);
    VG_HIP(hipStreamSynchronize(s));
    if (n_long > 0 && n_long <= LONG_CAP) {
        {
            vg_prof_scope ps("index_long_runs", 0);
            hipLaunchKernelGGL(k_long_groups, dim3(n_long), dim3(256), 0, s, si.keys.p, si.pos.p, g->d_blk2g.p, g->align_shift, nv, si.low_bit,
                               long_list.p, gen.p, rowinfo.p, cmap, d_dups.p, d_full.p);
        }
        d_full.download(&need_full, 1, s); d_dups.download(ix.dups.data(), (size_t)n, s);
        VG_HIP(hipStreamSynchronize(s));
    }
    if (need_full || n_long > LONG_CAP) {
        rowinfo.zero(s); d_dups.zero(s);
        finish_sort(si, k);
        {
            vg_prof_scope ps("index_runs_general", (double)nv * (8 + 4 + 4 + 8));
            hipLaunchKernelGGL(k_runs, dim3(grid_for((nv + 3) / 4)), dim3(256), 0, s, si.keys.p, si.pos.p, g->d_blk2g.p, g->align_shift, nv,
                               gen.p, rowinfo.p, cmap, d_dups.p);
        }
        d_dups.download(ix.dups.data(), (size_t)n, s);
        VG_HIP(hipStreamSynchronize(s));
    }
}
static void spgemm_pairs(vg_genomes* g, const kmer_index& ix, uint32_t min_shared, std::vector<vg_pair_count>& host_pairs,
                         dbuf<vg_pair_count>* dev_out, unsigned long long* dev_n, int first_row = 0) {
    hipStream_t s = vg_stream(); const int n = g->n;
    if (first_row >= n) { host_pairs.clear(); if (dev_out) { dev_out->alloc(1); *dev_n = 0; } return; }
    dbuf<unsigned long long> d_cursor(1);
    dbuf<uint32_t> d_over((size_t)n), d_nover(1);
    unsigned long long cap = std::max<unsigned long long>(1u << 20, (unsigned long long)n * 16);
    constexpr int64_t SMALL_ROW = 8192;
    dbuf<uint32_t> d_small, d_large; int n_small = 0, n_large = 0;
    if (n >= (1 << 16)) {
        std::vector<uint32_t> small_rows, large_rows;
        std::vector<uint32_t> goff_h;
        if (ix.rows_from_map) { goff_h.resize((size_t)n + 1); ix.si.goff.download(goff_h.data(), (size_t)n + 1, s); VG_HIP(hipStreamSynchronize(s)); }
        auto rows_of = [&](int i) { return !goff_h.empty() ? (int64_t)(goff_h[(size_t)i + 1] - goff_h[(size_t)i]) : ix.compact_rows ? (int64_t)ix.kept[(size_t)i] : g->len[(size_t)i]; };
        for (int i = first_row; i < n; ++i) (rows_of(i) <= SMALL_ROW ? small_rows : large_rows).push_back((uint32_t)i);
        if (small_rows.size() * 2 >= (size_t)(n - first_row)) {
            n_small = (int)small_rows.size(); n_large = (int)large_rows.size();
            d_small.alloc(small_rows.size()); d_small.upload(small_rows.data(), small_rows.size(), s);
            if (n_large) { d_large.alloc(large_rows.size()); d_large.upload(large_rows.data(), large_rows.size(), s); }
        }
    }
    dbuf<uint32_t> d_tail;
    if (first_row > 0 && !n_small) {
        std::vector<uint32_t> tail((size_t)(n - first_row));
        for (int i = first_row; i < n; ++i) tail[(size_t)(i - first_row)] = (uint32_t)i;
        d_tail.alloc(tail.size()); d_tail.upload(tail.data(), tail.size(), s);
        VG_HIP(hipStreamSynchronize(s));
    }
    for (;;) {
        dbuf<vg_pair_count> d_out((size_t)cap);
        d_cursor.zero(s); d_nover.zero(s);
        auto launch = [&](auto kern, int threads, const uint32_t* rows, int n_rows, uint32_t* over) {
            hipLaunchKernelGGL(kern, dim3((n_rows + 7) / 8 * 8), dim3(threads), 0, s, ix.rowinfo.p, ix.gen.p, (uint64_t)ix.gen.n, g->d_base_off.p, g->d_len.p, ix.wbase, n,
                               min_shared, rows, n_rows, d_out.p, d_cursor.p, cap, over, d_nover.p, ix.inline_lo);
        };
        {
            vg_prof_scope ps("spgemm_rows", (double)ix.n_rows_info * 4.0);
            if (n_small) {
                if (n_large) launch(k_spgemm<11>, 256, d_large.p, n_large, d_over.p);
                launch(k_spgemm<9, true>, 64, d_small.p, n_small, d_over.p);
            } else launch(k_spgemm<11>, 256, d_tail.p, n - first_row, d_over.p);
        }
        constexpr size_t EAGER = 1 << 16;
        uint32_t nover = 0; unsigned long long produced = 0;
        host_pairs.resize(dev_out ? 0 : std::min<size_t>(EAGER, (size_t)cap));
        d_nover.download(&nover, 1, s); d_cursor.download(&produced, 1, s);
        if (!dev_out) d_out.download(host_pairs.data(), host_pairs.size(), s);
        VG_HIP(hipStreamSynchronize(s));
        vg_host_mark("spgemm done");
        if (nover == 0 && produced <= (dev_out ? cap : host_pairs.size())) { if (dev_out) { *dev_out = std::move(d_out); *dev_n = produced; } else host_pairs.resize((size_t)produced); break; }
        if (nover > 0) {
            dbuf<uint32_t> d_rows2(nover), d_over2(nover);
            VG_HIP(hipMemcpyAsync(d_rows2.p, d_over.p, sizeof(uint32_t) * nover, hipMemcpyDeviceToDevice, s));
            d_nover.zero(s);
            {
                vg_prof_scope ps("spgemm_rows_wide", 0);
                launch(k_spgemm<13>, 256, d_rows2.p, (int)nover, d_over2.p);
            }
            VG_HIP(hipMemcpyAsync(d_over.p, d_over2.p, sizeof(uint32_t) * nover, hipMemcpyDeviceToDevice, s));
            d_nover.download(&nover, 1, s);
            VG_HIP(hipStreamSynchronize(s));
        }
        if (nover > 0) {
            std::vector<uint32_t> rows(nover); d_over.download(rows.data(), nover, s); VG_HIP(hipStreamSynchronize(s));
            const uint32_t batch = (uint32_t)std::max<int64_t>(1, std::min<int64_t>(nover, (int64_t)(1u << 28) / std::max(n, 1)));
            dbuf<uint32_t> dense((size_t)batch * n), d_rows(batch);
            for (uint32_t o = 0; o < nover; o += batch) {
                uint32_t nb = std::min(batch, nover - o);
                dense.zero(s);
                d_rows.upload(rows.data() + o, nb, s);
                vg_prof_scope ps("spgemm_dense_rows", 0);
                hipLaunchKernelGGL(k_spgemm_dense, dim3(nb), dim3(256), 0, s, ix.rowinfo.p, ix.gen.p, (uint64_t)ix.gen.n, g->d_base_off.p,
                                   g->d_len.p, ix.wbase, n, min_shared, d_rows.p, dense.p, d_out.p, d_cursor.p, cap, ix.inline_lo);
                VG_HIP(hipStreamSynchronize(s));
            }
        }
        d_cursor.download(&produced, 1, s);
        VG_HIP(hipStreamSynchronize(s));
        if (produced <= cap) {
            if (dev_out) { *dev_out = std::move(d_out); *dev_n = produced; break; }
            host_pairs.resize((size_t)produced);
            if (produced) d_out.download(host_pairs.data(), (size_t)produced, s);
            VG_HIP(hipStreamSynchronize(s));
            break;
        }
        cap = produced + produced / 8 + 1024;
    }
}
static bool pass_source_dense(int64_t P, double fraction, int n_shards, bool masked) {
    return !(fraction < 1.0) && (n_shards == 1 || range_shards(P, fraction, n_shards)) && !masked;
}
static void build_index(vg_genomes* g, int k, double fraction, int shard, int n_shards, const pass_inputs& in, kmer_index& ix) {
    ix.d_dups.alloc((size_t)g->n); ix.d_dups.zero(vg_stream());
    ix.kept.resize((size_t)g->n); ix.dups.resize((size_t)g->n);
    const bool range = range_shards(g, fraction, n_shards);
    const bool dense_src = pass_source_dense(g->padded_total(), fraction, n_shards, in.mask != nullptr);
    const bool bucket_ok = index_by_buckets(g, k, fraction, shard, n_shards, dense_src, in, ix);
    if (!bucket_ok) index_by_radix(g, k, fraction, shard, n_shards, in, ix);
    ix.compact_rows = bucket_ok ? (!dense_src || range) : ix.si.compact;
    ix.rows_from_map = in.xs && range && bucket_ok;
    ix.wbase = ix.compact_rows ? ix.si.wave_base.p : nullptr;
}
static void kmer_shared_pass(vg_genomes* g, int k, double fraction, int shard, int n_shards, uint32_t min_shared, int64_t* set_sizes, std::vector<vg_pair_count>& host_pairs,
                             const pass_inputs& in = pass_inputs{}, dbuf<vg_pair_count>* dev_out = nullptr, unsigned long long* dev_n = nullptr) {
    const int n = g->n;
    kmer_index ix;
    build_index(g, k, fraction, shard, n_shards, in, ix);
    for (int i = 0; i < n; ++i) set_sizes[i] = (int64_t)ix.kept[i] - ix.dups[i];
    ix.si.keys.release();
    if (in.pre && in.next_shard >= 0)
        try { vg_dev_try_scope opportunistic; launch_precount(*in.pre, g, k, in.next_shard, n_shards); } catch (...) { (void)hipGetLastError(); in.pre->drop(); }
    spgemm_pairs(g, ix, min_shared, host_pairs, dev_out, dev_n, in.first_row);
}

namespace {
__global__ void k_pair_keys(const vg_pair_count* __restrict__ rec, int64_t n, uint64_t* __restrict__ keys, uint32_t* __restrict__ vals) {
    for (int64_t i = (int64_t)blockIdx.x * blockDim.x + threadIdx.x; i < n; i += (int64_t)gridDim.x * blockDim.x) {
        const vg_pair_count r = rec[i]; keys[i] = ((uint64_t)r.a << 32) | r.b; vals[i] = r.shared;
    }
}
}
namespace {
__global__ void k_pair_keep(const uint32_t* __restrict__ sums, int64_t n, uint32_t min_shared, uint32_t* __restrict__ keep) {
    for (int64_t i = (int64_t)blockIdx.x * blockDim.x + threadIdx.x; i < n; i += (int64_t)gridDim.x * blockDim.x) keep[i] = sums[i] >= min_shared ? 1u : 0u;
}
__global__ void k_pair_place(const uint64_t* __restrict__ keys, const uint32_t* __restrict__ sums, const uint32_t* __restrict__ keep,
                             const uint32_t* __restrict__ at, int64_t n, vg_pair_count* __restrict__ out) {
    for (int64_t i = (int64_t)blockIdx.x * blockDim.x + threadIdx.x; i < n; i += (int64_t)gridDim.x * blockDim.x) {
        if (!keep[i]) continue;
        vg_pair_count r; r.a = (uint32_t)(keys[i] >> 32); r.b = (uint32_t)keys[i]; r.shared = sums[i];
        out[at[i]] = r;
    }
}
}
static void sum_partial_pairs(const std::vector<dbuf<vg_pair_count>>& parts, const std::vector<unsigned long long>& counts, uint32_t min_shared,
                              dbuf<vg_pair_count>& out, unsigned long long* n_out) {
    *n_out = 0;
    size_t n = 0; for (unsigned long long c : counts) n += (size_t)c;
    if (!n) return;
    if (n >= (1ull << 32)) throw vg_error(VG_EOVERFLOW, "more than 2^32 partial pair records in one call");
    hipStream_t s = vg_stream();
    dbuf<uint64_t> k1(n), k2(n), uk(n); dbuf<uint32_t> v1(n), v2(n), us(n); dbuf<unsigned long long> d_nu(1);
    size_t off = 0;
    for (size_t t = 0; t < parts.size(); ++t) {
        if (!counts[t]) continue;
        hipLaunchKernelGGL(k_pair_keys, dim3(grid_for((int64_t)counts[t])), dim3(256), 0, s, (const vg_pair_count*)parts[t].p, (int64_t)counts[t], k1.p + off, v1.p + off);
        off += (size_t)counts[t];
    }
    size_t tb = 0, tb2 = 0, tb3 = 0;
    VG_HIP(rocprim::radix_sort_pairs(nullptr, tb, k1.p, k2.p, v1.p, v2.p, n, 0u, 64u, s));
    VG_HIP(rocprim::reduce_by_key(nullptr, tb2, k2.p, v2.p, n, uk.p, us.p, d_nu.p, rocprim::plus<uint32_t>(), rocprim::equal_to<uint64_t>(), s));
    VG_HIP(rocprim::exclusive_scan(nullptr, tb3, v1.p, v2.p, 0u, n, rocprim::plus<uint32_t>(), s));
    dbuf<char> tmp(std::max(tb, std::max(tb2, tb3)));
    VG_HIP(rocprim::radix_sort_pairs((void*)tmp.p, tb, k1.p, k2.p, v1.p, v2.p, n, 0u, 64u, s));
    VG_HIP(rocprim::reduce_by_key((void*)tmp.p, tb2, k2.p, v2.p, n, uk.p, us.p, d_nu.p, rocprim::plus<uint32_t>(), rocprim::equal_to<uint64_t>(), s));
    unsigned long long nu = 0; d_nu.download(&nu, 1, s); VG_HIP(hipStreamSynchronize(s));
    if (!nu) return;
    hipLaunchKernelGGL(k_pair_keep, dim3(grid_for((int64_t)nu)), dim3(256), 0, s, (const uint32_t*)us.p, (int64_t)nu, min_shared, v1.p);
    VG_HIP(rocprim::exclusive_scan((void*)tmp.p, tb3, v1.p, v2.p, 0u, (size_t)nu, rocprim::plus<uint32_t>(), s));
    uint32_t last_at = 0, last_keep = 0;
    VG_HIP(hipMemcpyAsync(&last_at, v2.p + (nu - 1), sizeof(uint32_t), hipMemcpyDeviceToHost, s));
    VG_HIP(hipMemcpyAsync(&last_keep, v1.p + (nu - 1), sizeof(uint32_t), hipMemcpyDeviceToHost, s));
    VG_HIP(hipStreamSynchronize(s));
    const unsigned long long no = (unsigned long long)last_at + last_keep;
    out.alloc((size_t)std::max<unsigned long long>(no, 1));
    if (no) hipLaunchKernelGGL(k_pair_place, dim3(grid_for((int64_t)nu)), dim3(256), 0, s, (const uint64_t*)uk.p, (const uint32_t*)us.p, (const uint32_t*)v1.p,
                               (const uint32_t*)v2.p, (int64_t)nu, out.p);
    VG_HIP(hipStreamSynchronize(s));
    *n_out = no;
}
static bool subshards_share_scan(const vg_genomes* g, double fraction, int n_shards, int sub) {
    return !g_sw.scan_each && sub >= 2 && sub <= MM_MAX_SUB && !range_shards(g, fraction, n_shards * sub);
}
static void kmer_shared_subshards(vg_genomes* g, int k, double fraction, int shard, int n_shards, int sub, uint32_t min_shared,
                                  int64_t* set_sizes, dbuf<vg_pair_count>& out, unsigned long long* n_out, int first_row = 0) {
    const int n = g->n;
    std::vector<int64_t> part((size_t)n);
    for (int i = 0; i < n; ++i) set_sizes[i] = 0;
    std::vector<dbuf<vg_pair_count>> parts((size_t)sub); std::vector<unsigned long long> counts((size_t)sub, 0ULL);
    std::vector<vg_pair_count> none;
    precount ahead;
    dbuf<unsigned long long> all_masks;
    const int64_t Wm = g->padded_total() / 64 + 1;
    const bool multi = subshards_share_scan(g, fraction, n_shards, sub);
    if (multi) {
        int rc = vg_genomes_to_device(g); if (rc) throw vg_error(rc, vg_last_error());
        hipStream_t s = vg_stream();
        all_masks.alloc((size_t)sub * (size_t)Wm);
        const kmer_args A = make_kmer_args(g, k, fraction, 0, 1);
        const int64_t P = g->padded_total();
        const size_t lds = (size_t)4 * sub * 8 * sizeof(uint32_t);
        vg_prof_scope ps("kmer_multi_mask", (double)P * (3.0 / 8.0 + sub / 8.0));
        with_k(k == 25 && !A.use_frac, [&](auto K) { hipLaunchKernelGGL(k_multi_mask<K()>, dim3(grid_for((P + 255) / 4)), dim3(256), lds, s, A, (uint32_t)(shard * sub), (uint32_t)sub, (uint32_t)(n_shards * sub), all_masks.p, Wm); });
    }
    const bool scan_ahead = !multi && !(fraction < 1.0) && !range_shards(g, fraction, n_shards * sub);
    for (int t = 0; t < sub; ++t) {
        pass_inputs in; if (multi) in.mask = all_masks.p + (size_t)t * (size_t)Wm;
        in.first_row = first_row;
        if (scan_ahead) { in.pre = &ahead; in.next_shard = t + 1 < sub ? shard * sub + t + 1 : -1; }
        kmer_shared_pass(g, k, fraction, shard * sub + t, n_shards * sub, 1u, part.data(), none, in, &parts[(size_t)t], &counts[(size_t)t]);
        for (int i = 0; i < n; ++i) set_sizes[i] += part[i];
    }
    vg_host_mark("sub-shards done");
    sum_partial_pairs(parts, counts, min_shared, out, n_out);
}

struct shard_plan { int sub; bool one_pass, range, retry_finer; };
static shard_plan plan_shards(const vg_genomes* g, double fraction, int n_shards, bool host_entry) {
    const int64_t P = g->padded_total();
    int64_t real_bases = 0; for (int i = 0; i < g->n; ++i) real_bases += g->len[(size_t)i];
    const double expect = (double)real_bases * fraction / n_shards;
    const bool dense = fraction >= 1.0 && n_shards == 1;
    const bool too_large = dense ? P >= (1LL << 32) : expect >= SUB_PASS_START;
    const int forced = g_force_subshards > (host_entry ? 0 : 1) ? g_force_subshards : 0;
    int sub = 1;
    if (forced) sub = forced;
    else if (host_entry && g_sw.subshards > 0) sub = g_sw.subshards;
    else if (too_large) sub = std::max(2, (int)std::ceil(expect / SUB_PASS_KMERS));
    else if (host_entry && dense && vg_one_shot())
        sub = std::max(1, (int)std::min(64.0, std::ceil(16.0 * (double)P / (g_sw.workspace_gb * 1073741824.0))));
    return { sub, sub == 1, range_shards(g, fraction, n_shards * sub), !forced };
}

static std::mutex g_trials_mu;
static int g_placement_trials = 1;
static std::map<std::pair<int64_t, int>, int> g_trials_done;
static int placement_trials_now() {
    std::lock_guard<std::mutex> lk(g_trials_mu);
    return g_sw.placement_trials > 0 ? g_sw.placement_trials : g_placement_trials;
}
extern "C" void vg_set_placement_trials(int n) {
    std::lock_guard<std::mutex> lk(g_trials_mu);
    g_placement_trials = n < 1 ? 1 : (n > 8 ? 8 : n);
    g_trials_done.clear();
}
static void check_kmer_args(int k, double fraction = 1.0, int shard = 0, int n_shards = 1) {
    if (k < 8 || k > 31) throw vg_error(VG_EINVAL, "k out of range (8..31)");
    if (n_shards < 1 || shard < 0 || shard >= n_shards) throw vg_error(VG_EINVAL, "bad shard");
    if (!(fraction > 0.0) || fraction > 1.0) throw vg_error(VG_EINVAL, "fraction must be in (0,1]");
}
template <class T> static T* to_caller(const std::vector<T>& v) {
    T* out = (T*)malloc(sizeof(T) * std::max<size_t>(1, v.size()));
    if (!out) throw vg_error(VG_ENOMEM, "out of host memory");
    if (!v.empty()) memcpy(out, v.data(), sizeof(T) * v.size());
    return out;
}
struct shard_call {
    vg_genomes* g; int k; double fraction; int shard, n_shards; uint32_t min_shared;
    int first_row = 0;
    vg_slice_exchange* xs = nullptr;
};
static void run_passes(const shard_call& c, const shard_plan& plan, int64_t* set_sizes, std::vector<vg_pair_count>& host_pairs,
                       dbuf<vg_pair_count>* dev_pairs = nullptr, unsigned long long* dev_n = nullptr) {
    if (plan.one_pass) {
        pass_inputs in; in.xs = c.xs; in.first_row = c.first_row;
        return kmer_shared_pass(c.g, c.k, c.fraction, c.shard, c.n_shards, c.min_shared, set_sizes, host_pairs, in, dev_pairs, dev_n);
    }
    dbuf<vg_pair_count> d_sum; unsigned long long n_sum = 0;
    dbuf<vg_pair_count>& sum = dev_pairs ? *dev_pairs : d_sum;
    for (int attempt = 0, sub = plan.sub;; ++attempt) {
        try { kmer_shared_subshards(c.g, c.k, c.fraction, c.shard, c.n_shards, sub, c.min_shared, set_sizes, sum, &n_sum, c.first_row); break; }
        catch (const vg_error& e) { if (e.code != VG_EOVERFLOW || attempt >= 3 || !plan.retry_finer) throw; ++sub; sum.release(); }
    }
    if (dev_pairs) { *dev_n = n_sum; return; }
    host_pairs.resize((size_t)n_sum);
    if (n_sum) { d_sum.download(host_pairs.data(), (size_t)n_sum, vg_stream()); VG_HIP(hipStreamSynchronize(vg_stream())); }
}
static void placement_trials(const shard_call& c) {
    vg_genomes* g = c.g; const int k = c.k, n = g->n;
    const int64_t P = g->padded_total(); const bool dense = c.fraction >= 1.0 && c.n_shards == 1;
    const int max_trials = placement_trials_now();
    size_t fr = 0, tot = 0;
    bool first_time = false;
    if (dense && !vg_one_shot() && max_trials > 1 && P >= (1LL << 30)) {
        std::lock_guard<std::mutex> lk(g_trials_mu);
        first_time = !g_trials_done[{ P, k }]++;
    }
    if (!(first_time && hipMemGetInfo(&fr, &tot) == hipSuccess && fr > 2 * vg_dev_cached_bytes() + (8ULL << 30))) return;
    float index_ms = 0.f; pass_inputs timed; timed.index_ms = &index_ms;
    std::vector<int64_t> sz2((size_t)n); std::vector<vg_pair_count> acc2;
    auto pass = [&] { kmer_shared_pass(g, k, c.fraction, c.shard, c.n_shards, c.min_shared, sz2.data(), acc2, timed); };
    float best = 0.f;
    try {
        pass();
        best = index_ms;
    } catch (...) { (void)hipGetLastError(); best = 0.f; }
    for (int trial = 1; trial < max_trials && best > 0.f; ++trial) {
        const double w0 = vg_alloc_wait_ms();
        vg_dev_park_cache();
        bool keep_new = false;
        try {
            pass();
            pass();
            keep_new = index_ms > 0.f && index_ms < 0.97f * best;
            if (getenv("VG_ALLOC_TRACE")) fprintf(stderr, "[vg placement] trial %d: index stage %.2f ms against %.2f ms -> %s\n", trial, index_ms, best, keep_new ? "kept" : "dropped");
            if (keep_new) best = index_ms;
        } catch (...) { (void)hipGetLastError(); keep_new = false; }
        vg_dev_unpark(!keep_new);
        if (vg_alloc_wait_ms() - w0 > 500.0) break;
    }
}
extern "C" int vg_kmer_shared(vg_genomes* g, int k, double fraction, int shard, int n_shards, uint32_t min_shared,
                              int64_t* set_sizes, vg_pair_count** pairs, int64_t* n_pairs) {
    VG_API_BEGIN
    if (!g || !set_sizes || !pairs || !n_pairs) throw vg_error(VG_EINVAL, "vg_kmer_shared: null argument");
    check_kmer_args(k, fraction, shard, n_shards);
    vg_host_mark("vg_kmer_shared: enter");
    vg_require_device();
    int rc = vg_genomes_to_device(g); if (rc) return rc;
    *pairs = nullptr; *n_pairs = 0;
    if (g->n == 0) return VG_OK;
    const shard_plan plan = plan_shards(g, fraction, n_shards, true);
    shard_call call{ g, k, fraction, shard, n_shards, min_shared };
    vg_slice_exchange xs; xs.rank = shard; xs.world = n_shards; xs.emulate = true;
    if (plan.one_pass && g_range_scan_mode == 1 && vg_slice_exchange_applies(g, k, fraction, n_shards)) call.xs = &xs;
    std::vector<vg_pair_count> acc;
    run_passes(call, plan, set_sizes, acc);
    if (plan.one_pass) placement_trials(call);
    vg_host_mark("pass done");
    *pairs = to_caller(acc); *n_pairs = (int64_t)acc.size();
    vg_host_mark("vg_kmer_shared: return");
    VG_API_END
}

namespace {
constexpr int NM_BITS = 19;
struct new_mask_args {
    const uint32_t* rec; int short_kr;
    const uint32_t* T1s; const uint32_t* off1;
    int nb1; int64_t n_st, st_pos;
    int64_t p_new, st_new, P;
    int chunks;
    const uint32_t* blk2g; int align_shift; const uint8_t* flag;
};
template <bool BY_GENOME>
__global__ void __launch_bounds__(PT_THREADS)
k_new_mask(new_mask_args a, unsigned long long* __restrict__ mask) {
    __shared__ uint32_t bits[BY_GENOME ? 1 : 1 << (NM_BITS - 5)];
    const int b = (int)(blockIdx.x / (unsigned)a.chunks), c = (int)(blockIdx.x % (unsigned)a.chunks);
    const int wave = threadIdx.x >> 6, lane = threadIdx.x & 63, n_waves = PT_THREADS / 64;
    auto segment = [&](int64_t st, uint32_t* r0, uint32_t* r1) {
        *r0 = a.T1s[st * a.nb1 + b];
        *r1 = st + 1 < a.n_st ? a.T1s[(st + 1) * a.nb1 + b] : a.off1[b + 1];
    };
    auto record = [&](uint32_t i, int64_t st, uint64_t* key, uint32_t* pos) {
        if (a.short_kr > 0) {
            uint64_t r; __builtin_memcpy(&r, a.rec + 2 * (size_t)i, 8);
            *key = short_rec_key(r);
            *pos = short_group_base((uint64_t)st * (uint64_t)a.st_pos) + short_rec_low(r);
        } else {
            const uint32_t* r = a.rec + 3 * (size_t)i;
            *key = ((uint64_t)r[0] << 32) | r[1]; *pos = r[2];
        }
    };
    auto keep = [&](uint32_t pos) { atomicOr(&mask[pos >> 6], 1ULL << (pos & 63u)); };
    if (BY_GENOME) {
        for (int64_t st = (int64_t)c * n_waves + wave; st < a.n_st; st += (int64_t)a.chunks * n_waves) {
            uint32_t r0, r1; segment(st, &r0, &r1);
            for (uint32_t i = r0 + lane; i < r1; i += 64) {
                uint64_t key; uint32_t pos; record(i, st, &key, &pos);
                if ((int64_t)pos < a.P && a.flag[a.blk2g[pos >> a.align_shift]]) keep(pos);
            }
        }
        return;
    }
    for (int i = threadIdx.x; i < (1 << (NM_BITS - 5)); i += PT_THREADS) bits[i] = 0;
    __syncthreads();
    for (int64_t st = a.st_new + wave; st < a.n_st; st += n_waves) {
        uint32_t r0, r1; segment(st, &r0, &r1);
        for (uint32_t i = r0 + lane; i < r1; i += 64) {
            uint64_t key; uint32_t pos; record(i, st, &key, &pos);
            if ((int64_t)pos < a.p_new || (int64_t)pos >= a.P) continue;
            const uint32_t h = (uint32_t)((key * 0x9E3779B97F4A7C15ULL) >> (64 - NM_BITS));
            atomicOr(&bits[h >> 5], 1u << (h & 31u));
            if (c == 0) keep(pos);
        }
    }
    __syncthreads();
    for (int64_t st = (int64_t)c * n_waves + wave; st <= a.st_new; st += (int64_t)a.chunks * n_waves) {
        uint32_t r0, r1; segment(st, &r0, &r1);
        for (uint32_t i = r0 + lane; i < r1; i += 64) {
            uint64_t key; uint32_t pos; record(i, st, &key, &pos);
            if ((int64_t)pos >= a.p_new) continue;
            const uint32_t h = (uint32_t)((key * 0x9E3779B97F4A7C15ULL) >> (64 - NM_BITS));
            if ((bits[h >> 5] >> (h & 31u)) & 1u) keep(pos);
        }
    }
}
}
static int g_new_path = 0;
extern "C" void vg_set_new_path(int mode) { g_new_path = mode == 1 || mode == 2 ? mode : 0; }
constexpr double NEW_MASKED_UP_TO = 0.01;
constexpr double NEW_SIZES_SHARE = 0.25; constexpr int64_t NEW_SIZES_FEW = 4096;
static bool kmer_shared_new_masked(vg_genomes* g, int n_db, int k, uint32_t min_shared, int64_t* set_sizes, std::vector<vg_pair_count>& acc) {
    hipStream_t s = vg_stream(); const int n = g->n; const int64_t P = g->padded_total();
    if (n_db <= 0 || n_db >= n || P >= (1LL << 32)) return false;
    const kmer_args A = make_kmer_args(g, k, 1.0, 0, 1);
    kmer_index ix1; pass_inputs none; dbuf<int> kept_b((size_t)n); kept_b.zero(s);
    ix1.n_rows_info = P;
    bucket_run R{ g, k, true, none, ix1, kept_b.p, s };
    if (open_bucket_run(R, A, [](bucket_run&) {}) != level1::records) return false;
    const bucket_geometry& G = R.G;
    new_mask_args a{};
    a.rec = R.a_rec.p; a.short_kr = G.short_rec ? G.L2.kr : 0; a.T1s = R.T1s.p; a.off1 = R.d_off1.p;
    a.nb1 = G.nb1; a.n_st = G.n_st; a.st_pos = (int64_t)G.st_tiles * PT_TILE;
    a.p_new = g->base_off[(size_t)n_db]; a.st_new = a.p_new / a.st_pos; a.P = P;
    a.blk2g = g->d_blk2g.p; a.align_shift = g->align_shift;
    const double new_share = (double)(P - a.p_new) / (double)P;
    const int64_t groups = (a.st_new + PT_THREADS / 64) / (PT_THREADS / 64);
    a.chunks = (int)std::max<int64_t>(1, std::min<int64_t>(std::min<int64_t>(groups, 64), (int64_t)((1.0 - new_share) / (8.0 * std::max(new_share, 1e-6)))));
    const int64_t W = P / 64;
    dbuf<unsigned long long> mask((size_t)W + 1); mask.zero(s);
    {
        vg_prof_scope ps("kmer_new_mask", (double)R.n1 * (G.short_rec ? 8.0 : 12.0));
        hipLaunchKernelGGL(k_new_mask<false>, dim3((unsigned)(G.nb1 * a.chunks)), dim3(PT_THREADS), 0, s, a, mask.p);
    }
    pass_inputs in; in.mask = mask.p; in.first_row = n_db;
    std::vector<int64_t> sizes((size_t)n); std::vector<vg_pair_count> pairs;
    kmer_shared_pass(g, k, 1.0, 0, 1, min_shared, sizes.data(), pairs, in);
    std::vector<uint8_t> flag((size_t)n, 0); int64_t n_flag = 0;
    for (const vg_pair_count& pc : pairs) if ((int64_t)pc.b < n_db && !flag[pc.b]) { flag[pc.b] = 1; ++n_flag; }
    if (n_flag > NEW_SIZES_FEW && (double)n_flag > NEW_SIZES_SHARE * n_db) return false;
    if (n_flag) {
        dbuf<uint8_t> d_flag((size_t)n); d_flag.upload(flag.data(), (size_t)n, s);
        mask.zero(s);
        a.flag = d_flag.p; a.chunks = (int)std::max<int64_t>(1, std::min<int64_t>(64, (a.n_st + PT_THREADS / 64 - 1) / (PT_THREADS / 64)));
        {
            vg_prof_scope ps("kmer_new_sizes", (double)R.n1 * (G.short_rec ? 8.0 : 12.0));
            hipLaunchKernelGGL(k_new_mask<true>, dim3((unsigned)(G.nb1 * a.chunks)), dim3(PT_THREADS), 0, s, a, mask.p);
        }
        VG_HIP(hipStreamSynchronize(s));
        kmer_index ix2; pass_inputs in2; in2.mask = mask.p;
        build_index(g, k, 1.0, 0, 1, in2, ix2);
        for (int i = 0; i < n_db; ++i) if (flag[(size_t)i]) sizes[(size_t)i] = (int64_t)ix2.kept[(size_t)i] - ix2.dups[(size_t)i];
    }
    for (int i = 0; i < n; ++i) set_sizes[i] = sizes[(size_t)i];
    acc.swap(pairs);
    return true;
}

extern "C" int vg_kmer_shared_new(vg_genomes* g, int n_db, int k, double fraction, uint32_t min_shared,
                                  int64_t* set_sizes, vg_pair_count** pairs, int64_t* n_pairs) {
    VG_API_BEGIN
    if (!g || !set_sizes || !pairs || !n_pairs) throw vg_error(VG_EINVAL, "vg_kmer_shared_new: null argument");
    check_kmer_args(k, fraction);
    if (n_db < 0 || n_db > g->n)
        throw vg_error(VG_EINVAL, "vg_kmer_shared_new: n_db = " + std::to_string(n_db) + " is outside 0.." + std::to_string(g->n) + " (the genomes of the set)");
    vg_host_mark("vg_kmer_shared_new: enter");
    vg_require_device();
    int rc = vg_genomes_to_device(g); if (rc) return rc;
    *pairs = nullptr; *n_pairs = 0;
    const int n = g->n;
    if (n == 0) return VG_OK;
    const shard_plan plan = plan_shards(g, fraction, 1, true);
    std::vector<vg_pair_count> acc;
    const int64_t P = g->padded_total();
    const bool want_masked = g_new_path == 2 || (g_new_path == 0 && n_db < n && (double)(P - g->base_off[(size_t)n_db]) <= NEW_MASKED_UP_TO * (double)P);
    bool masked_done = false;
    if (plan.one_pass && fraction >= 1.0 && want_masked)
        try { masked_done = kmer_shared_new_masked(g, n_db, k, min_shared, set_sizes, acc); }
        catch (const vg_error& e) { if (e.code != VG_EOVERFLOW) throw; acc.clear(); }
    if (!masked_done) run_passes(shard_call{ g, k, fraction, 0, 1, min_shared, n_db }, plan, set_sizes, acc);
    std::vector<char> named((size_t)n_db, 0);
    for (const vg_pair_count& pc : acc) if ((int64_t)pc.b < n_db) named[(size_t)pc.b] = 1;
    for (int i = 0; i < n_db; ++i) if (!named[(size_t)i]) set_sizes[i] = -1;
    *pairs = to_caller(acc); *n_pairs = (int64_t)acc.size();
    vg_host_mark("vg_kmer_shared_new: return");
    VG_API_END
}

int vg_kmer_shard_mode(const vg_genomes* g, double fraction, int n_shards) { return plan_shards(g, fraction, n_shards, false).range ? 1 : 2; }
void vg_kmer_shared_device(vg_genomes* g, int k, double fraction, int shard, int n_shards, uint32_t min_shared,
                           int64_t* set_sizes, dbuf<vg_pair_count>& pairs, int64_t* n_pairs, vg_slice_exchange* xs, int* mode_out) {
    if (mode_out) *mode_out = 0;
    vg_require_device();
    int rc = vg_genomes_to_device(g); if (rc) throw vg_error(rc, vg_last_error());
    *n_pairs = 0;
    if (g->n == 0) return;
    const shard_plan plan = plan_shards(g, fraction, n_shards, false);
    if (mode_out) *mode_out = plan.range ? 1 : 2;
    unsigned long long n = 0; std::vector<vg_pair_count> none;
    run_passes(shard_call{ g, k, fraction, shard, n_shards, min_shared, 0, xs }, plan, set_sizes, none, &pairs, &n);
    if (!plan.one_pass && !pairs.p) pairs.alloc(1);
    *n_pairs = (int64_t)n;
}

static_assert(sizeof(vg_pair_count) == 12, "pair record layout");
extern "C" void vg_set_subshards(int n) { g_force_subshards = n; }
extern "C" void vg_set_range_scan(int mode) { g_range_scan_mode = mode == 1 ? 1 : 0; }

static void report_geometry(int k, bool dense, const kmer_args& A, int64_t P, vg_kmer_geometry_info* info) {
    bucket_geometry G;
    info->accepted = dense ? (bucket_geometry_for(k, true, A, P, G) ? 1 : 0) : -1;
    if (info->accepted != 1) return;
    info->levels = G.levels; info->total_bits = G.total_bits; info->B1 = G.B1; info->B2 = G.B2;
    info->st_tiles = G.st_tiles; info->n_st = G.n_st; info->u_st = G.L2.u_st; info->g_st = G.L2.g_st;
    info->tile32k = G.tile32k; info->narrow = G.narrow; info->short_rec = G.short_rec;
}
extern "C" int vg_kmer_geometry(const vg_genomes* g, int k, double fraction, int shard, int n_shards, vg_kmer_geometry_info* info) {
    VG_API_BEGIN
    if (!g || !info) throw vg_error(VG_EINVAL, "vg_kmer_geometry: null argument");
    check_kmer_args(k, fraction, shard, n_shards);
    memset(info, 0, sizeof *info);
    const int64_t P = g->padded_total();
    info->P = P; info->n_passes = 1;
    if (g->n == 0) return VG_OK;
    const shard_plan plan = plan_shards(g, fraction, n_shards, true);
    info->n_passes = plan.sub;
    const int sh = shard * plan.sub, ns = n_shards * plan.sub;
    const bool masked = subshards_share_scan(g, fraction, n_shards, plan.sub);
    const bool dense = pass_source_dense(P, fraction, ns, masked);
    report_geometry(k, dense, shard_kmer_args(P, g->align_shift, k, 1.0, sh, ns), P, info);
    VG_API_END
}
extern "C" int vg_kmer_geometry_at(int64_t padded_positions, int k, vg_kmer_geometry_info* info) {
    VG_API_BEGIN
    if (!info) throw vg_error(VG_EINVAL, "vg_kmer_geometry_at: null argument");
    check_kmer_args(k);
    if (padded_positions < 0) throw vg_error(VG_EINVAL, "vg_kmer_geometry_at: negative number of positions");
    memset(info, 0, sizeof *info);
    info->P = padded_positions; info->n_passes = 1;
    report_geometry(k, true, shard_kmer_args(padded_positions, 0, k, 1.0, 0, 1), padded_positions, info);
    VG_API_END
}
extern "C" int vg_rowptr_inline_lo(int64_t entries, int64_t n_genomes, uint32_t* inline_lo) {
    VG_API_BEGIN
    if (!inline_lo) throw vg_error(VG_EINVAL, "vg_rowptr_inline_lo: null argument");
    if (entries < 0 || n_genomes < 0) throw vg_error(VG_EINVAL, "vg_rowptr_inline_lo: negative count");
    *inline_lo = rowptr_inline_lo((uint64_t)entries, n_genomes);
    VG_API_END
}

extern "C" int vg_kmer_set(vg_genomes* g, int idx, int k, double fraction, uint64_t** out, int64_t* n_out) {
    VG_API_BEGIN
    if (!g || !out || !n_out || idx < 0 || idx >= g->n) throw vg_error(VG_EINVAL, "vg_kmer_set: bad argument");
    check_kmer_args(k, fraction);
    vg_require_device();
    int rc = vg_genomes_to_device(g); if (rc) return rc;
    hipStream_t s = vg_stream();
    sorted_index si;
    extract_kmers(g, k, fraction, 0, 1, pass_inputs{}, si);
    prefix_sort(si, k);
    finish_sort(si, k);
    std::vector<uint64_t> keys((size_t)si.n_valid); std::vector<uint32_t> pos((size_t)si.n_valid);
    if (si.n_valid) { si.keys.download(keys.data(), keys.size(), s); si.pos.download(pos.data(), pos.size(), s); }
    VG_HIP(hipStreamSynchronize(s));
    std::vector<uint64_t> mine;
    int64_t lo = g->base_off[idx], hi = g->base_off[idx + 1];
    if (si.compact) {
        uint32_t c[2];
        VG_HIP(hipMemcpyAsync(&c[0], si.wave_base.p + (lo >> 6), sizeof(uint32_t), hipMemcpyDeviceToHost, s));
        VG_HIP(hipMemcpyAsync(&c[1], si.wave_base.p + (hi >> 6), sizeof(uint32_t), hipMemcpyDeviceToHost, s));
        VG_HIP(hipStreamSynchronize(s));
        lo = c[0]; hi = c[1];
    }
    for (size_t i = 0; i < keys.size(); ++i)
        if ((int64_t)pos[i] >= lo && (int64_t)pos[i] < hi) {
            const uint64_t hl = unscramble_key(keys[i], k), H = hl >> k, L = hl & ((1ULL << k) - 1ULL);
            uint64_t x = 0;
            for (int b = 0; b < k; ++b) x |= ((((H >> b) & 1ULL) << 1) | ((L >> b) & 1ULL)) << (2 * b);
            mine.push_back(cano_codes_of(x, k));
        }
    std::sort(mine.begin(), mine.end());
    mine.erase(std::unique(mine.begin(), mine.end()), mine.end());
// ... 7 lines not shown
```

Measured before the change: 2.761 million.

## Group LZ tasks on host with pinned staging and keep small plans device-side

Replaces the GPU counting, radix sort and record kernels for grouping align tasks with a multithreaded host count and scatter into a reused pinned buffer, uploaded asynchronously on a side stream after the first index batch is queued. Small single-batch LZ plans now keep their device buffers between calls so descriptors and indexes need not be re-uploaded. The prefilter hands its realloc-backed pair buffer straight to the caller instead of copying it, and skips re-downloading pairs already fetched. These target per-call launch, sync, allocation and copy overheads, at the cost of more host CPU work and device memory held across calls.

```diff
diff --git a/include/vclust_gpu.h b/include/vclust_gpu.h
--- a/include/vclust_gpu.h
+++ b/include/vclust_gpu.h
@@ -101,6 +101,8 @@
 
 int vg_align_tasks(const vg_genomes* g, const vg_pair_count* pairs, int64_t n_pairs,
                    vg_task** tasks, int64_t* n_tasks);
+int vg_lz_group_tasks_host(const vg_task* tasks, int64_t n_tasks, int n_genomes, int n_threads,
+                           uint32_t* records, uint32_t* ref_ids, int64_t* n_refs, int64_t* ref_first);
 int vg_lz_index_dump(vg_genomes* g, int idx, const vg_lz_params* p,
                      uint32_t** bucket_end, uint32_t** entries, int64_t* n_entries,
                      int* pos_bits, int* tag_bits, int* path);
diff --git a/vclust_amd/_lib.py b/vclust_amd/_lib.py
--- a/vclust_amd/_lib.py
+++ b/vclust_amd/_lib.py
@@ -171,6 +171,7 @@
     'vg_read_filter': (C.c_int, [C.c_void_p, C.c_char_p, C.c_double, P(P(PairCount)), P(C.c_int64)]),
     'vg_align_tasks': (C.c_int, [C.c_void_p, P(PairCount), C.c_int64, P(P(Task)), P(C.c_int64)]),
     'vg_lz_prepare': (C.c_int, [C.c_void_p, P(PairCount), C.c_int64, P(LzParams)]),
+    'vg_lz_group_tasks_host': (C.c_int, [P(Task), C.c_int64, C.c_int, C.c_int, P(C.c_uint32), P(C.c_uint32), P(C.c_int64), P(C.c_int64)]),
     'vg_lz_index_dump': (C.c_int, [C.c_void_p, C.c_int, P(LzParams), P(P(C.c_uint32)), P(P(C.c_uint32)), P(C.c_int64),
                                    P(C.c_int), P(C.c_int), P(C.c_int)]),
     'vg_set_index_budget': (None, [C.c_int64]),
diff --git a/vclust_amd/build.py b/vclust_amd/build.py
--- a/vclust_amd/build.py
+++ b/vclust_amd/build.py
@@ -29,7 +29,7 @@
 
 def build_lib(force: bool = False, verbose: bool = False) -> pathlib.Path:
     srcs = [CSRC / s for s in SOURCES]
-    deps = srcs + [CSRC / 'vg_common.h', CSRC / 'vg_window.h', ROOT / 'include' / 'vclust_gpu.h']
+    deps = srcs + [CSRC / 'vg_common.h', CSRC / 'vg_window.h', CSRC / 'vg_group.h', ROOT / 'include' / 'vclust_gpu.h']
     if not force and not _stale(LIB_PATH, deps):
         return LIB_PATH
     obj_dir = PKG_DIR / '_obj'
@@ -44,7 +44,7 @@
     for s in srcs:
         o = obj_dir / (s.name + '.o')
         objs.append(o)
-        if force or _stale(o, [s, CSRC / 'vg_common.h', CSRC / 'vg_window.h', ROOT / 'include' / 'vclust_gpu.h']):
+        if force or _stale(o, [s, CSRC / 'vg_common.h', CSRC / 'vg_window.h', CSRC / 'vg_group.h', ROOT / 'include' / 'vclust_gpu.h']):
             cmd = [hipcc, *flags, '-x', 'hip', '-c', str(s), '-o', str(o)]
             if verbose:
                 print(' '.join(cmd), file=sys.stderr)
diff --git a/vclust_amd/csrc/vg_align.hip b/vclust_amd/csrc/vg_align.hip
--- a/vclust_amd/csrc/vg_align.hip
+++ b/vclust_amd/csrc/vg_align.hip
@@ -1,5 +1,6 @@
 #include "vg_common.h"
 #include "vg_window.h"
+#include "vg_group.h"
 #include <rocprim/rocprim.hpp>
 #include <algorithm>
 #include <numeric>
@@ -894,7 +895,6 @@
     }
 }
 
-struct task_dev { uint32_t q, r_slot, out_idx, pad; };
 
 constexpr int SEG_LOG_CAP = 250;
 constexpr int PW_AFTER_EVENT = 32;
@@ -1234,42 +1234,6 @@
 static bool g_index_budget_set = false;
 static int64_t g_index_budget_bytes = [] { const char* e = getenv("VG_INDEX_BUDGET_GB"); const double v = e ? atof(e) : 0.0; g_index_budget_set = v >= 0.0625; return v >= 0.0625 ? (int64_t)(v * 1073741824.0) : (24LL << 30); }();
 namespace {
-__global__ void __launch_bounds__(256)
-k_task_count(const vg_task* __restrict__ tasks, int64_t n_tasks, int n_genomes, const int64_t* __restrict__ len,
-             uint32_t* __restrict__ ref_cnt, uint32_t* __restrict__ keys, uint32_t* __restrict__ vals,
-             unsigned long long* __restrict__ sums ) {
-    unsigned long long sq = 0, sr = 0, mq = 0, bad = 0;
-    for (int64_t t = (int64_t)blockIdx.x * blockDim.x + threadIdx.x; t < n_tasks; t += (int64_t)gridDim.x * blockDim.x) {
-        const vg_task tk = tasks[t];
-        keys[t] = tk.r; vals[t] = (uint32_t)t;
-        if (tk.q >= (uint32_t)n_genomes || tk.r >= (uint32_t)n_genomes) { bad = 1; continue; }
-        atomicAdd(&ref_cnt[tk.r], 1u);
-        const unsigned long long ql = (unsigned long long)len[tk.q];
-        sq += ql; sr += (unsigned long long)len[tk.r]; mq = ql > mq ? ql : mq;
-    }
-    for (int o = 32; o > 0; o >>= 1) {
-        sq += __shfl_xor(sq, o); sr += __shfl_xor(sr, o); bad |= __shfl_xor(bad, o);
-        const unsigned long long m2 = __shfl_xor(mq, o); mq = m2 > mq ? m2 : mq;
-    }
-    if ((threadIdx.x & 63) == 0) {
-        if (sq) atomicAdd(&sums[0], sq);
-        if (sr) atomicAdd(&sums[1], sr);
-        if (mq) atomicMax(&sums[2], mq);
-        if (bad) atomicOr(&sums[3], 1ULL);
-    }
-}
-__global__ void __launch_bounds__(256)
-k_task_records(const vg_task* __restrict__ tasks, const uint32_t* __restrict__ sorted_idx, int64_t n_tasks,
-               const uint32_t* __restrict__ ord , task_dev* __restrict__ td) {
-    for (int64_t i = (int64_t)blockIdx.x * blockDim.x + threadIdx.x; i < n_tasks; i += (int64_t)gridDim.x * blockDim.x) {
-        const uint32_t t = sorted_idx[i];
-        const vg_task tk = tasks[t];
-        td[i] = { tk.q, ord[tk.r], t, 0u };
-    }
-}
-}
-
-namespace {
 struct lz_batch {
     int first_ref = 0, n_refs = 0;
     std::vector<int64_t> chunk_off{ 0 };
@@ -1287,6 +1251,7 @@
     lz_slot slot;
     int64_t budget = 0; int mal = 0, msl = 0; const vg_genomes* g = nullptr; int n_genomes = 0;
     bool batch0_built = false;
+    bool dev_side = false;
 };
 int64_t lz_batch_budget(const vg_genomes* g, const vg_lz_params* p, const std::vector<uint32_t>& ref_ids);
 void lz_plan_references(const vg_genomes* g, const vg_lz_params* p, lz_plan& P);
@@ -1294,7 +1259,33 @@
 void lz_build_batch(const vg_genomes* g, const vg_lz_params* p, lz_plan& P, size_t bi, hipStream_t sb);
 std::mutex g_prep_mu;
 std::unique_ptr<lz_plan> g_prepared;
+constexpr size_t PLAN_DEV_KEEP = 64u << 20;
 std::unique_ptr<lz_plan> g_plan_cache;
+struct lz_task_stage {
+    task_dev* pin = nullptr; size_t cap = 0; dbuf<task_dev> dev;
+    hipEvent_t uploaded = nullptr, released = nullptr; bool copy_pending = false;
+    lz_task_stage() {
+        VG_HIP(hipEventCreateWithFlags(&uploaded, hipEventDisableTiming));
+        if (hipEventCreateWithFlags(&released, hipEventDisableTiming) != hipSuccess) { (void)hipEventDestroy(uploaded); throw vg_error(VG_EHIP, "hipEventCreate failed"); }
+    }
+    lz_task_stage(const lz_task_stage&) = delete; lz_task_stage& operator=(const lz_task_stage&) = delete;
+    ~lz_task_stage() {
+        if (copy_pending) (void)hipEventSynchronize(uploaded);
+        if (pin) (void)hipHostFree(pin);
+        (void)hipEventDestroy(uploaded); (void)hipEventDestroy(released);
+    }
+    bool reserve(size_t n) {
+        if (copy_pending) { VG_HIP(hipEventSynchronize(uploaded)); copy_pending = false; }
+        if (n <= cap) return false;
+        if (pin) { (void)hipHostFree(pin); pin = nullptr; } cap = 0;
+        dev.release();
+        const size_t want = n + n / 8;
+        VG_HIP(hipHostMalloc((void**)&pin, want * sizeof(task_dev), hipHostMallocPortable));
+        dev.alloc(want); cap = want;
+        return true;
+    }
+};
+std::unique_ptr<lz_task_stage> g_task_stage;
 std::unique_ptr<lz_plan> lz_take_plan(std::unique_ptr<lz_plan>& kept, const vg_genomes* g, const vg_lz_params* p, const std::vector<uint32_t>& ref_ids) {
     std::lock_guard<std::mutex> lk(g_prep_mu);
     std::unique_ptr<lz_plan> Q = std::move(kept);
@@ -1312,18 +1303,28 @@
     }
     return plan;
 }
-void lz_keep_plan_host_side(std::unique_ptr<lz_plan>& plan) {
+void lz_keep_plan(std::unique_ptr<lz_plan>& plan) {
     if (!plan || vg_one_shot()) return;
-    plan->slot = lz_slot(); plan->d_refs.release();
+    lz_slot& L = plan->slot;
+    L.rr_pool.release(); L.mask_pool.release(); L.stab_pool.release(); L.sent_pool.release(); L.scratch.release();
+    const size_t dev_bytes = plan->d_refs.bytes() + L.d_reg.bytes() + L.d_mid.bytes() + L.d_small.bytes() + L.d_large.bytes() + L.d_lchunk.bytes();
+    plan->dev_side = plan->batches.size() == 1 && plan->batch0_built && dev_bytes <= PLAN_DEV_KEEP;
+    if (!plan->dev_side) { plan->slot = lz_slot(); plan->d_refs.release(); }
     plan->batch0_built = false;
     std::lock_guard<std::mutex> lk(g_prep_mu);
     g_plan_cache = std::move(plan);
 }
 }
+namespace {
+void lz_drop_prepared_plan(const vg_genomes* g) {
+    if (g_prepared && (!g || g_prepared->g == g)) { (void)hipStreamSynchronize(vg_stream()); g_prepared.reset(); }
+}
+}
 void vg_lz_drop_prepared(const vg_genomes* g) {
     std::lock_guard<std::mutex> lk(g_prep_mu);
-    if (g_prepared && (!g || g_prepared->g == g)) { (void)hipStreamSynchronize(vg_stream()); g_prepared.reset(); }
+    lz_drop_prepared_plan(g);
     if (g_plan_cache && (!g || g_plan_cache->g == g)) g_plan_cache.reset();
+    if (!g) g_task_stage.reset();
 }
 
 namespace {
@@ -1373,42 +1374,40 @@
 }
 
 struct lz_tasks {
-    dbuf<task_dev> d_tasks;
-    std::vector<int64_t> ref_first;
-    std::vector<uint32_t> ref_ids;
+    lz_task_counts C;
+    const task_dev* d_tasks = nullptr;
+    const task_dev* td = nullptr;
     int64_t q_max = 0; double q_sum = 0, bytes_alg_all = 0;
-    std::vector<task_dev> td;
 };
-lz_tasks lz_group_tasks(const vg_genomes* g, const vg_task* tasks, int64_t n_tasks, bool host_copy, hipStream_t s) {
-    lz_tasks T;
-    T.ref_first.assign((size_t)g->n + 1, 0);
-    T.d_tasks.alloc((size_t)n_tasks);
-    dbuf<vg_task> d_raw((size_t)n_tasks); d_raw.upload(tasks, (size_t)n_tasks, s);
-    dbuf<uint32_t> d_cnt((size_t)g->n), d_keys((size_t)n_tasks), d_vals((size_t)n_tasks), d_keys2((size_t)n_tasks), d_vals2((size_t)n_tasks);
-    dbuf<unsigned long long> d_sums(4);
-    d_cnt.zero(s); d_sums.zero(s);
-    hipLaunchKernelGGL(k_task_count, dim3(grid_for(n_tasks, 256, 512)), dim3(256), 0, s,
-                       (const vg_task*)d_raw.p, n_tasks, g->n, g->d_len.p, d_cnt.p, d_keys.p, d_vals.p, d_sums.p);
-    std::vector<uint32_t> cnt((size_t)g->n); unsigned long long sums[4];
-    d_cnt.download(cnt.data(), cnt.size(), s); d_sums.download(sums, 4, s);
-    const unsigned id_bits = bit_width((uint64_t)std::max(g->n, 1) - 1, 1);
-    with_temp_storage([&](void* tmp, size_t& tb) {
-        return rocprim::radix_sort_pairs(tmp, tb, d_keys.p, d_keys2.p, d_vals.p, d_vals2.p, (size_t)n_tasks, 0u, id_bits, s); });
-    VG_HIP(hipStreamSynchronize(s));
-    if (sums[3]) throw vg_error(VG_EINVAL, "task id out of range");
-    std::vector<uint32_t> ord((size_t)g->n, 0);
-    for (int i = 0; i < g->n; ++i) {
-        if (cnt[(size_t)i]) { ord[(size_t)i] = (uint32_t)T.ref_ids.size(); T.ref_ids.push_back((uint32_t)i); }
-        T.ref_first[(size_t)i + 1] = T.ref_first[(size_t)i] + cnt[(size_t)i];
-    }
-    T.q_max = (int64_t)sums[2]; T.q_sum = (double)sums[0];
-    T.bytes_alg_all = ((double)sums[0] + (double)sums[1]) / 4.0 + 20.0 * (double)n_tasks;
-    dbuf<uint32_t> d_ord((size_t)g->n); d_ord.upload(ord.data(), ord.size(), s);
-    hipLaunchKernelGGL(k_task_records, dim3(grid_for(n_tasks)), dim3(256), 0, s, (const vg_task*)d_raw.p, (const uint32_t*)d_vals2.p, n_tasks,
-                       (const uint32_t*)d_ord.p, T.d_tasks.p);
-    if (host_copy) { T.td.resize((size_t)n_tasks); T.d_tasks.download(T.td.data(), T.td.size(), s); }
-    VG_HIP(hipStreamSynchronize(s));
-    return T;
+void lz_count(const vg_genomes* g, const vg_task* tasks, int64_t n_tasks, lz_tasks& T) {
+    lz_count_tasks(tasks, n_tasks, g->n, g->len.data(), vg_host_threads(), T.C);
+    T.q_max = (int64_t)T.C.max_q; T.q_sum = (double)T.C.sum_q;
+    T.bytes_alg_all = ((double)T.C.sum_q + (double)T.C.sum_r) / 4.0 + 20.0 * (double)n_tasks;
+}
+struct lz_stage_hold {
+    std::unique_ptr<lz_task_stage> st; hipStream_t s;
+    explicit lz_stage_hold(hipStream_t lib) : s(lib) {
+        { std::lock_guard<std::mutex> lk(g_prep_mu); st = std::move(g_task_stage); }
+        if (!st) st.reset(new lz_task_stage);
+    }
+    ~lz_stage_hold() {
+        (void)hipEventRecord(st->released, s);
+        if (vg_one_shot()) return;
+        std::lock_guard<std::mutex> lk(g_prep_mu);
+        if (!g_task_stage) g_task_stage = std::move(st);
+    }
+};
+void lz_stage_tasks(lz_task_stage& st, const vg_task* tasks, int64_t n_tasks, lz_tasks& T, hipStream_t s) {
+    const bool fresh = st.reserve((size_t)n_tasks);
+    lz_scatter_tasks(tasks, n_tasks, T.C, vg_host_threads(), st.pin);
+    vg_host_mark("lz: tasks grouped");
+    hipStream_t up = vg_side_stream();
+    if (fresh) VG_HIP(hipEventRecord(st.released, s));
+    VG_HIP(hipStreamWaitEvent(up, st.released, 0));
+    VG_HIP(hipMemcpyAsync(st.dev.p, st.pin, (size_t)n_tasks * sizeof(task_dev), hipMemcpyHostToDevice, up));
+    VG_HIP(hipEventRecord(st.uploaded, up)); st.copy_pending = true;
+    VG_HIP(hipStreamWaitEvent(s, st.uploaded, 0));
+    T.d_tasks = st.dev.p; T.td = st.pin;
 }
 
 struct lz_kernel_params { lz_dev_params P; bool fast; };
@@ -1427,7 +1426,8 @@
 struct lz_range { int64_t pos, end; double bytes_alg; int64_t q_max, q_sum; };
 lz_range lz_task_range(const lz_batch& B, const lz_tasks& T, int64_t n_tasks) {
     const size_t ri_end = (size_t)B.first_ref + (size_t)B.n_refs;
-    const int64_t pos = T.ref_first[T.ref_ids[(size_t)B.first_ref]], end = ri_end < T.ref_ids.size() ? T.ref_first[T.ref_ids[ri_end]] : n_tasks;
+    const std::vector<int64_t>& ref_first = T.C.ref_first; const std::vector<uint32_t>& ref_ids = T.C.ref_ids;
+    const int64_t pos = ref_first[ref_ids[(size_t)B.first_ref]], end = ri_end < ref_ids.size() ? ref_first[ref_ids[ri_end]] : n_tasks;
     return { pos, end, T.bytes_alg_all * (double)(end - pos) / (double)n_tasks, T.q_max, (int64_t)(T.q_sum * (double)(end - pos) / (double)n_tasks) };
 }
 
@@ -1503,7 +1503,7 @@
     if (used > cap && lz_parse_and_place(c, R, c.fast, used, misplaced, h_regions) > used)
         throw vg_error(VG_EHIP, "internal error: the region arena of the LZ parse overflowed twice");
 }
-void lz_batch_two_pass(const lz_call& c, const lz_range& R, const std::vector<task_dev>& td, std::vector<vg_pair_stat>& first_pass, std::vector<vg_region>& h_regions) {
+void lz_batch_two_pass(const lz_call& c, const lz_range& R, const task_dev* td, std::vector<vg_pair_stat>& first_pass, std::vector<vg_region>& h_regions) {
     { vg_prof_scope ps("lz_parse", R.bytes_alg); lz_launch_parse(c, R, false, c.fast); }
     std::vector<vg_pair_stat> h_stats((size_t)c.n_tasks);
     vg_download_bytes(h_stats.data(), c.d_stats, h_stats.size() * sizeof(vg_pair_stat), c.s);
@@ -1540,21 +1540,25 @@
     if (n_tasks >= (1LL << 32)) throw vg_error(VG_EOVERFLOW, "more than 2^32 - 1 ordered pairs in one call: split the task list");
     const bool want_regions = regions != nullptr, two_pass = want_regions && g_sw.two_pass;
 
-    const lz_tasks T = lz_group_tasks(g, tasks, n_tasks, two_pass, s);
-    vg_host_mark("lz: tasks grouped");
+    lz_tasks T;
+    lz_count(g, tasks, n_tasks, T);
+    vg_host_mark("lz: tasks counted");
     const lz_kernel_params K = lz_device_params(g, p);
     dbuf<vg_pair_stat> d_stats((size_t)n_tasks);
-    std::unique_ptr<lz_plan> plan = lz_take_plan(g_prepared, g, p, T.ref_ids);
-    if (!plan) plan = lz_plan_for(g, p, T.ref_ids);
+    std::unique_ptr<lz_plan> plan = lz_take_plan(g_prepared, g, p, T.C.ref_ids);
+    if (!plan) plan = lz_plan_for(g, p, T.C.ref_ids);
     std::vector<lz_range> ranges;
     for (const lz_batch& B : plan->batches) ranges.push_back(lz_task_range(B, T, n_tasks));
     vg_host_mark("lz: batches planned");
-
-    const lz_call c{ g, d_planes, T.d_tasks.p, plan.get(), K.P, K.fast, d_stats.p, n_tasks, s };
+    if (!plan->batch0_built) { lz_build_batch(g, p, *plan, 0, s); plan->batch0_built = true; vg_host_mark("lz: first batch of indexes queued"); }
+    lz_stage_hold stage(s);
+    lz_stage_tasks(*stage.st, tasks, n_tasks, T, s);
+
+    const lz_call c{ g, d_planes, T.d_tasks, plan.get(), K.P, K.fast, d_stats.p, n_tasks, s };
     std::vector<vg_region> h_regions;
     std::vector<vg_pair_stat> first_pass;
     for (size_t bi = 0; bi < ranges.size(); ++bi) {
-        if (!(bi == 0 && plan->batch0_built)) lz_build_batch(g, p, *plan, bi, s);
+        if (bi > 0) lz_build_batch(g, p, *plan, bi, s);
         if (!want_regions) lz_batch_rows(c, ranges[bi]);
         else if (two_pass) lz_batch_two_pass(c, ranges[bi], T.td, first_pass, h_regions);
         else lz_batch_regions(c, ranges[bi], h_regions);
@@ -1576,7 +1580,7 @@
         if (!h_regions.empty()) memcpy(o, h_regions.data(), sizeof(vg_region) * h_regions.size());
         *regions = o; if (n_regions) *n_regions = (int64_t)h_regions.size();
     }
-    lz_keep_plan_host_side(plan);
+    lz_keep_plan(plan);
     VG_API_END
 }
 
@@ -1681,9 +1685,11 @@
     hipStream_t s = vg_stream();
     std::vector<lz_batch>& batches = P.batches;
     std::vector<ref_desc>& all_refs = P.all_refs;
-    P.d_refs.alloc(std::max<size_t>(1, all_refs.size()));
-    if (!all_refs.empty()) P.d_refs.upload(all_refs.data(), all_refs.size(), s);
-    vg_host_mark("lz plan: descriptors queued");
+    if (!P.dev_side) {
+        P.d_refs.alloc(std::max<size_t>(1, all_refs.size()));
+        if (!all_refs.empty()) P.d_refs.upload(all_refs.data(), all_refs.size(), s);
+        vg_host_mark("lz plan: descriptors queued");
+    }
     size_t m_rr = 0, m_mask = 0, m_stab = 1, m_sent = 0, m_scr = 1, m_reg = 1, m_mid = 1, m_small = 1, m_large = 1, m_lch = 1;
     for (auto& B : batches) {
         m_rr = std::max(m_rr, (size_t)B.rr_words); m_mask = std::max(m_mask, (size_t)B.mask_words);
@@ -1693,16 +1699,19 @@
     }
     lz_slot& L = P.slot;
     L.rr_pool.alloc(m_rr + 8); L.mask_pool.alloc(m_mask + 8); L.stab_pool.alloc(m_stab); L.sent_pool.alloc(m_sent + 4);
-    L.scratch.alloc(m_scr); L.d_reg.alloc(m_reg); L.d_mid.alloc(m_mid); L.d_small.alloc(m_small); L.d_large.alloc(m_large); L.d_lchunk.alloc(m_lch);
+    L.scratch.alloc(m_scr);
+    if (!P.dev_side) { L.d_reg.alloc(m_reg); L.d_mid.alloc(m_mid); L.d_small.alloc(m_small); L.d_large.alloc(m_large); L.d_lchunk.alloc(m_lch); }
 }
 void lz_build_batch(const vg_genomes* g, const vg_lz_params* p, lz_plan& P, size_t bi, hipStream_t sb) {
     lz_batch& B = P.batches[bi];
     lz_slot& L = P.slot;
     dbuf<ref_desc>& d_refs = P.d_refs;
-    if (!B.reg_list.empty()) L.d_reg.upload(B.reg_list.data(), B.reg_list.size(), sb);
-    if (!B.mid_list.empty()) L.d_mid.upload(B.mid_list.data(), B.mid_list.size(), sb);
-    if (!B.small_list.empty()) L.d_small.upload(B.small_list.data(), B.small_list.size(), sb);
-    if (!B.large_list.empty()) { L.d_large.upload(B.large_list.data(), B.large_list.size(), sb); L.d_lchunk.upload(B.large_chunks.data(), B.large_chunks.size(), sb); }
+    if (!P.dev_side) {
+        if (!B.reg_list.empty()) L.d_reg.upload(B.reg_list.data(), B.reg_list.size(), sb);
+        if (!B.mid_list.empty()) L.d_mid.upload(B.mid_list.data(), B.mid_list.size(), sb);
+        if (!B.small_list.empty()) L.d_small.upload(B.small_list.data(), B.small_list.size(), sb);
+        if (!B.large_list.empty()) { L.d_large.upload(B.large_list.data(), B.large_list.size(), sb); L.d_lchunk.upload(B.large_chunks.data(), B.large_chunks.size(), sb); }
+    }
     const int64_t total_chunks = B.chunk_off.back();
     const uint32_t* gpl = vg_genome_planes(g, sb);
     vg_prof_scope ps("lz_build_index", (double)total_chunks * 32 * (0.375 + 0.375 + 4), sb);
@@ -1745,7 +1754,7 @@
     lz_check_params(p);
     vg_require_device();
     int rc = vg_genomes_to_device(g); if (rc) return rc;
-    vg_lz_drop_prepared(nullptr);
+    { std::lock_guard<std::mutex> lk(g_prep_mu); lz_drop_prepared_plan(nullptr); }
     if (n_pairs == 0) return VG_OK;
     lz_check_lengths(g, 0, g->n);
     std::vector<uint8_t> is_ref((size_t)g->n, 0);
diff --git a/vclust_amd/csrc/vg_group.h b/vclust_amd/csrc/vg_group.h
--- /dev/null
+++ b/vclust_amd/csrc/vg_group.h
@@ -0,0 +1,61 @@
+#pragma once
+#include "vg_common.h"
+
+struct task_dev { uint32_t q, r_slot, out_idx, pad; };
+
+struct lz_task_counts {
+    std::vector<int64_t> ref_first;
+    std::vector<uint32_t> ref_ids;
+    std::vector<uint32_t> ord;
+    uint64_t sum_q = 0, sum_r = 0, max_q = 0;
+};
+
+namespace vg_group_detail {
+inline int threads_for(int64_t n_tasks, int n_thr) { return n_tasks < (1 << 15) ? 1 : std::max(1, std::min(n_thr, 16)); }
+template <class F> void each_thread(int T, F fn) { if (T == 1) fn(0); else vg_parallel_for(T, T, [&](int64_t t) { fn((int)t); }); }
+}
+
+inline void lz_count_tasks(const vg_task* tasks, int64_t n_tasks, int n_genomes, const int64_t* len, int n_thr, lz_task_counts& C) {
+    const int64_t n = std::max(n_genomes, 0);
+    const int T = vg_group_detail::threads_for(n_tasks, n_thr);
+    C.ref_first.assign((size_t)n + 1, 0);
+    C.ref_ids.clear(); C.ord.assign((size_t)n, 0);
+    std::vector<uint64_t> part((size_t)T * 4, 0);
+    int64_t* const cnt = C.ref_first.data() + 1;
+    vg_group_detail::each_thread(T, [&](int t) {
+        const uint32_t lo = (uint32_t)(n * t / T), span = (uint32_t)(n * (t + 1) / T) - lo;
+        for (int64_t i = 0; i < n_tasks; ++i) { const uint32_t d = tasks[i].r - lo; if (d < span) cnt[lo + d]++; }
+        uint64_t sq = 0, sr = 0, mq = 0, bad = 0;
+        for (int64_t i = n_tasks * t / T, e = n_tasks * (t + 1) / T; i < e; ++i) {
+            const vg_task tk = tasks[i];
+            if (tk.q >= (uint32_t)n || tk.r >= (uint32_t)n) { bad = 1; continue; }
+            if (len) { const uint64_t ql = (uint64_t)len[tk.q]; sq += ql; sr += (uint64_t)len[tk.r]; mq = std::max(mq, ql); }
+        }
+        uint64_t* p = &part[(size_t)t * 4]; p[0] = sq; p[1] = sr; p[2] = mq; p[3] = bad;
+    });
+    uint64_t bad = 0;
+    C.sum_q = C.sum_r = C.max_q = 0;
+    for (int t = 0; t < T; ++t) { const uint64_t* p = &part[(size_t)t * 4]; C.sum_q += p[0]; C.sum_r += p[1]; C.max_q = std::max(C.max_q, p[2]); bad |= p[3]; }
+    if (bad) throw vg_error(VG_EINVAL, "task id out of range");
+    for (int64_t r = 0; r < n; ++r) {
+        if (cnt[r]) { C.ord[(size_t)r] = (uint32_t)C.ref_ids.size(); C.ref_ids.push_back((uint32_t)r); }
+        C.ref_first[(size_t)r + 1] += C.ref_first[(size_t)r];
+    }
+}
+
+inline void lz_scatter_tasks(const vg_task* tasks, int64_t n_tasks, const lz_task_counts& C, int n_thr, task_dev* out) {
+    const int64_t n = (int64_t)C.ord.size();
+    const int T = vg_group_detail::threads_for(n_tasks, n_thr);
+    std::vector<int64_t> cur(C.ref_first.begin(), C.ref_first.end() - 1);
+    auto bound = [&](int t) { return t >= T ? n : (int64_t)(std::lower_bound(C.ref_first.begin(), C.ref_first.begin() + n, n_tasks * t / T) - C.ref_first.begin()); };
+    vg_group_detail::each_thread(T, [&](int t) {
+        const int64_t b0 = t == 0 ? 0 : bound(t), b1 = bound(t + 1);
+        const uint32_t lo = (uint32_t)b0, span = (uint32_t)(b1 - b0);
+        if (!span) return;
+        for (int64_t i = 0; i < n_tasks; ++i) {
+            const vg_task tk = tasks[i];
+            const uint32_t d = tk.r - lo;
+            if (d < span) out[cur[(size_t)tk.r]++] = { tk.q, C.ord[tk.r], (uint32_t)i, 0u };
+        }
+    });
+}
diff --git a/vclust_amd/csrc/vg_io.cpp b/vclust_amd/csrc/vg_io.cpp
--- a/vclust_amd/csrc/vg_io.cpp
+++ b/vclust_amd/csrc/vg_io.cpp
@@ -1,4 +1,5 @@
 #include "vg_common.h"
+#include "vg_group.h"
 #include <cmath>
 #include <math.h>
 #include <stdio.h>
@@ -357,6 +358,20 @@
     auto o = host_array<vg_pair_count>(v.size());
     if (!v.empty()) memcpy(o.get(), v.data(), sizeof(vg_pair_count) * v.size());
     *pairs = o.release(); *n_pairs = (int64_t)v.size();
+    VG_API_END
+}
+
+extern "C" int vg_lz_group_tasks_host(const vg_task* tasks, int64_t n_tasks, int n_genomes, int n_threads,
+                                      uint32_t* records, uint32_t* ref_ids, int64_t* n_refs, int64_t* ref_first) {
+    VG_API_BEGIN
+    if ((!tasks && n_tasks) || (!records && n_tasks) || !ref_ids || !n_refs || !ref_first || n_tasks < 0 || n_genomes < 0 || n_tasks >= (1LL << 32))
+        throw vg_error(VG_EINVAL, "vg_lz_group_tasks_host: bad argument");
+    static_assert(sizeof(task_dev) == 4 * sizeof(uint32_t), "a record is four words");
+    lz_task_counts C;
+    lz_count_tasks(tasks, n_tasks, n_genomes, nullptr, n_threads, C);
+    lz_scatter_tasks(tasks, n_tasks, C, n_threads, (task_dev*)records);
+    std::copy(C.ref_ids.begin(), C.ref_ids.end(), ref_ids); *n_refs = (int64_t)C.ref_ids.size();
+    std::copy(C.ref_first.begin(), C.ref_first.end(), ref_first);
     VG_API_END
 }
 
diff --git a/vclust_amd/csrc/vg_prefilter.hip b/vclust_amd/csrc/vg_prefilter.hip
--- a/vclust_amd/csrc/vg_prefilter.hip
+++ b/vclust_amd/csrc/vg_prefilter.hip
@@ -2371,7 +2371,28 @@
         VG_HIP(hipStreamSynchronize(s));
     }
 }
-static void spgemm_pairs(vg_genomes* g, const kmer_index& ix, uint32_t min_shared, std::vector<vg_pair_count>& host_pairs,
+struct pair_block {
+    vg_pair_count* p = nullptr; size_t n = 0, cap = 0;
+    pair_block() {}
+    pair_block(const pair_block&) = delete; pair_block& operator=(const pair_block&) = delete;
+    ~pair_block() { free(p); }
+    void resize(size_t m) {
+        if (m > cap) {
+            void* q = realloc(p, sizeof(vg_pair_count) * m);
+            if (!q) throw vg_error(VG_ENOMEM, "out of host memory");
+            p = (vg_pair_count*)q; cap = m;
+        }
+        n = m;
+    }
+    void clear() { n = 0; }
+    void swap(pair_block& o) { std::swap(p, o.p); std::swap(n, o.n); std::swap(cap, o.cap); }
+    vg_pair_count* data() { return p; }
+    size_t size() const { return n; }
+    const vg_pair_count* begin() const { return p; }
+    const vg_pair_count* end() const { return p + n; }
+    vg_pair_count* release() { if (!p) resize(1); vg_pair_count* q = p; p = nullptr; n = cap = 0; return q; }
+};
+static void spgemm_pairs(vg_genomes* g, const kmer_index& ix, uint32_t min_shared, pair_block& host_pairs,
                          dbuf<vg_pair_count>* dev_out, unsigned long long* dev_n, int first_row = 0) {
     hipStream_t s = vg_stream(); const int n = g->n;
     if (first_row >= n) { host_pairs.clear(); if (dev_out) { dev_out->alloc(1); *dev_n = 0; } return; }
@@ -2420,6 +2441,7 @@
         if (!dev_out) d_out.download(host_pairs.data(), host_pairs.size(), s);
         VG_HIP(hipStreamSynchronize(s));
         vg_host_mark("spgemm done");
+        const size_t eager_final = nover == 0 ? host_pairs.size() : 0;
         if (nover == 0 && produced <= (dev_out ? cap : host_pairs.size())) { if (dev_out) { *dev_out = std::move(d_out); *dev_n = produced; } else host_pairs.resize((size_t)produced); break; }
         if (nover > 0) {
             dbuf<uint32_t> d_rows2(nover), d_over2(nover);
@@ -2451,8 +2473,9 @@
         VG_HIP(hipStreamSynchronize(s));
         if (produced <= cap) {
             if (dev_out) { *dev_out = std::move(d_out); *dev_n = produced; break; }
+            const size_t have = std::min<size_t>(eager_final, (size_t)produced);
             host_pairs.resize((size_t)produced);
-            if (produced) d_out.download(host_pairs.data(), (size_t)produced, s);
+            if (produced > have) vg_download_bytes(host_pairs.data() + have, d_out.p + have, ((size_t)produced - have) * sizeof(vg_pair_count), s);
             VG_HIP(hipStreamSynchronize(s));
             break;
         }
@@ -2473,7 +2496,7 @@
     ix.rows_from_map = in.xs && range && bucket_ok;
     ix.wbase = ix.compact_rows ? ix.si.wave_base.p : nullptr;
 }
-static void kmer_shared_pass(vg_genomes* g, int k, double fraction, int shard, int n_shards, uint32_t min_shared, int64_t* set_sizes, std::vector<vg_pair_count>& host_pairs,
+static void kmer_shared_pass(vg_genomes* g, int k, double fraction, int shard, int n_shards, uint32_t min_shared, int64_t* set_sizes, pair_block& host_pairs,
                              const pass_inputs& in = pass_inputs{}, dbuf<vg_pair_count>* dev_out = nullptr, unsigned long long* dev_n = nullptr) {
     const int n = g->n;
     kmer_index ix;
@@ -2550,7 +2573,7 @@
     std::vector<int64_t> part((size_t)n);
     for (int i = 0; i < n; ++i) set_sizes[i] = 0;
     std::vector<dbuf<vg_pair_count>> parts((size_t)sub); std::vector<unsigned long long> counts((size_t)sub, 0ULL);
-    std::vector<vg_pair_count> none;
+    pair_block none;
     precount ahead;
     dbuf<unsigned long long> all_masks;
     const int64_t Wm = g->padded_total() / 64 + 1;
@@ -2622,7 +2645,7 @@
     int first_row = 0;
     vg_slice_exchange* xs = nullptr;
 };
-static void run_passes(const shard_call& c, const shard_plan& plan, int64_t* set_sizes, std::vector<vg_pair_count>& host_pairs,
+static void run_passes(const shard_call& c, const shard_plan& plan, int64_t* set_sizes, pair_block& host_pairs,
                        dbuf<vg_pair_count>* dev_pairs = nullptr, unsigned long long* dev_n = nullptr) {
     if (plan.one_pass) {
         pass_inputs in; in.xs = c.xs; in.first_row = c.first_row;
@@ -2650,7 +2673,7 @@
     }
     if (!(first_time && hipMemGetInfo(&fr, &tot) == hipSuccess && fr > 2 * vg_dev_cached_bytes() + (8ULL << 30))) return;
     float index_ms = 0.f; pass_inputs timed; timed.index_ms = &index_ms;
-    std::vector<int64_t> sz2((size_t)n); std::vector<vg_pair_count> acc2;
+    std::vector<int64_t> sz2((size_t)n); pair_block acc2;
     auto pass = [&] { kmer_shared_pass(g, k, c.fraction, c.shard, c.n_shards, c.min_shared, sz2.data(), acc2, timed); };
     float best = 0.f;
     try {
@@ -2686,11 +2709,11 @@
     shard_call call{ g, k, fraction, shard, n_shards, min_shared };
     vg_slice_exchange xs; xs.rank = shard; xs.world = n_shards; xs.emulate = true;
     if (plan.one_pass && g_range_scan_mode == 1 && vg_slice_exchange_applies(g, k, fraction, n_shards)) call.xs = &xs;
-    std::vector<vg_pair_count> acc;
+    pair_block acc;
     run_passes(call, plan, set_sizes, acc);
     if (plan.one_pass) placement_trials(call);
     vg_host_mark("pass done");
-    *pairs = to_caller(acc); *n_pairs = (int64_t)acc.size();
+    *n_pairs = (int64_t)acc.size(); *pairs = acc.release();
     vg_host_mark("vg_kmer_shared: return");
     VG_API_END
 }
@@ -2764,7 +2787,7 @@
 extern "C" void vg_set_new_path(int mode) { g_new_path = mode == 1 || mode == 2 ? mode : 0; }
 constexpr double NEW_MASKED_UP_TO = 0.01;
 constexpr double NEW_SIZES_SHARE = 0.25; constexpr int64_t NEW_SIZES_FEW = 4096;
-static bool kmer_shared_new_masked(vg_genomes* g, int n_db, int k, uint32_t min_shared, int64_t* set_sizes, std::vector<vg_pair_count>& acc) {
+static bool kmer_shared_new_masked(vg_genomes* g, int n_db, int k, uint32_t min_shared, int64_t* set_sizes, pair_block& acc) {
     hipStream_t s = vg_stream(); const int n = g->n; const int64_t P = g->padded_total();
     if (n_db <= 0 || n_db >= n || P >= (1LL << 32)) return false;
     const kmer_args A = make_kmer_args(g, k, 1.0, 0, 1);
@@ -2788,7 +2811,7 @@
         hipLaunchKernelGGL(k_new_mask<false>, dim3((unsigned)(G.nb1 * a.chunks)), dim3(PT_THREADS), 0, s, a, mask.p);
     }
     pass_inputs in; in.mask = mask.p; in.first_row = n_db;
-    std::vector<int64_t> sizes((size_t)n); std::vector<vg_pair_count> pairs;
+    std::vector<int64_t> sizes((size_t)n); pair_block pairs;
     kmer_shared_pass(g, k, 1.0, 0, 1, min_shared, sizes.data(), pairs, in);
     std::vector<uint8_t> flag((size_t)n, 0); int64_t n_flag = 0;
     for (const vg_pair_count& pc : pairs) if ((int64_t)pc.b < n_db && !flag[pc.b]) { flag[pc.b] = 1; ++n_flag; }
@@ -2825,7 +2848,7 @@
     const int n = g->n;
     if (n == 0) return VG_OK;
     const shard_plan plan = plan_shards(g, fraction, 1, true);
-    std::vector<vg_pair_count> acc;
+    pair_block acc;
     const int64_t P = g->padded_total();
     const bool want_masked = g_new_path == 2 || (g_new_path == 0 && n_db < n && (double)(P - g->base_off[(size_t)n_db]) <= NEW_MASKED_UP_TO * (double)P);
     bool masked_done = false;
@@ -2836,7 +2859,7 @@
     std::vector<char> named((size_t)n_db, 0);
     for (const vg_pair_count& pc : acc) if ((int64_t)pc.b < n_db) named[(size_t)pc.b] = 1;
     for (int i = 0; i < n_db; ++i) if (!named[(size_t)i]) set_sizes[i] = -1;
-    *pairs = to_caller(acc); *n_pairs = (int64_t)acc.size();
+    *n_pairs = (int64_t)acc.size(); *pairs = acc.release();
     vg_host_mark("vg_kmer_shared_new: return");
     VG_API_END
 }
@@ -2851,7 +2874,7 @@
     if (g->n == 0) return;
     const shard_plan plan = plan_shards(g, fraction, n_shards, false);
     if (mode_out) *mode_out = plan.range ? 1 : 2;
-    unsigned long long n = 0; std::vector<vg_pair_count> none;
+    unsigned long long n = 0; pair_block none;
     run_passes(shard_call{ g, k, fraction, shard, n_shards, min_shared, 0, xs }, plan, set_sizes, none, &pairs, &n);
     if (!plan.one_pass && !pairs.p) pairs.alloc(1);
     *n_pairs = (int64_t)n;
```

Result: slower. 2.724 million (-1.3%).
